# Geunwoo-Jeon/LarvaNet

Hardware: AMD Instinct MI355X
Metric: HR Mpixels/s (LarvaNet x4 multi-exit train step, 48x48 LR patches) (higher is better)
Workload: dtype f32; 1 GPU; LarvaNet x4 train_step_larva M4 B4,4,4,4 48ch, batch 16 of 3x48x48 -> 3x192x192 fp32 per GPU (BASELINE config 2); global_batch=16, parallelism=dp1, hip_graph=True

## Files before the change

### include/larva_hip.h

```cpp
#ifndef LARVA_HIP_H
#define LARVA_HIP_H

#include <stdint.h>

#ifdef __cplusplus
extern "C" {
#endif

int larva_abi_version(void);
const char* larva_error_string(int code);

long long larva_packed_weight_floats(int cout, int cin);
int larva_pack_weights(const float* w, float* wpk_fwd, float* wpk_bwd, int cout, int cin,
                       int w_cin_total, int w_cin_off, void* stream);

int larva_pack_weights_batch(const float* const* w, float* const* wpk_fwd, float* const* wpk_bwd,
                             const int* cout, const int* cin, const int* w_cin_total,
                             const int* w_cin_off, int njobs, void* stream);

int larva_step_prologue(const float* const* w, float* const* wpk_fwd, float* const* wpk_bwd, const int* cout,
                        const int* cin, const int* w_cin_total, const int* w_cin_off, int njobs, const float* x,
                        float* x16, float* base, int N, int C, int H, int W, void* stream);

int larva_conv3x3_fwd(const float* const* src, int n_src, int cin_per_src, const float* wpk,
                      const float* bias, const float* res0, const float* res1, const float* mask,
                      const float* base, float* out, int N, int cout, int H, int W, int relu,
                      int mode, void* stream);

int larva_conv3x3_fwd_pitched(const float* const* src, int n_src, int cin_per_src, const float* wpk,
                              const float* bias, const float* res0, const float* res1, const float* mask,
                              const float* base, float* out, int N, int cout, int H, int W, int pitch,
                              int relu, int mode, void* stream);

int larva_conv3x3_fwd_batch(int njobs, const float* const* src, int n_src, int cin_per_src,
                            const float* const* wpk, const float* const* bias, const float* const* res0,
                            const float* const* res1, const float* const* mask, const float* const* base,
                            float* const* out, int N, int cout, int H, int W, int pitch, int relu, int mode,
                            void* stream);

int larva_head_conv3_direct(const float* x, const float* w, const float* bias, float* out, int N, int cout,
                            int H, int W, int pitch, void* stream);

int larva_exit_l1_partials(int N, int H, int pitch);
int larva_conv3x3_exit_l1_batch(int njobs, const float* const* src, int n_src, int cin_per_src,
                                const float* const* wpk, const float* const* bias, const float* const* base,
                                const float* const* truth, float* const* out, float* const* grad,
                                float* const* partial, float gval, int N, int cout, int H, int W, int pitch,
                                void* stream);

int larva_strip_tile_table(int H, int W, int phase, unsigned* tab, int cap);
int larva_conv3x3_fwd_strips(const float* const* src, int n_src, int cin_per_src, const float* wpk,
                             const float* bias, const float* res0, const float* res1, const float* mask,
                             const float* base, float* out, int N, int cout, int H, int W, int pitch,
                             int relu, int mode, const unsigned* tile_tab, const unsigned* tile_tab_host,
                             int tiles_per_image, int plain_stores, void* stream);

int larva_conv3x3_fwd_tiled(const float* const* src, int n_src, int cin_per_src, const float* wpk,
                            const float* bias, const float* res0, const float* res1, const float* mask,
                            const float* base, float* out, int N, int cout, int H, int W, int pitch,
                            int relu, int mode, int tile_rows, void* stream);

long long larva_wgrad_partial_floats(int cout, int cin, int splits);
int larva_wgrad_cu_share(int cout, int cin);
int larva_conv3x3_wgrad(const float* const* dy, const float* const* x, float* const* partial,
                        float* const* dw, float* const* db, const int* cin_off,
                        const int* cin_valid, const int* w_cin_total, int njobs, int splits,
                        int N, int cout, int cin, int H, int W, void* stream);

int larva_wgrad_flat_max_splits(int njobs, int nwg, int tiles_per_layer);
int larva_conv3x3_wgrad_partial_flat(const float* const* dy, const float* const* x, float* const* partial,
                                     int njobs, int nwg, int N, int cout, int cin, int H, int W,
                                     int* splits_out, void* stream);
int larva_wgrad_flat_head_splits(int njobs, int nwg, int tiles_per_layer);
int larva_conv3x3_wgrad_partial_flat_head(const float* const* dy, const float* const* x, float* const* partial,
                                          int njobs, const float* head_dy, const float* head_x16, float* head_partial,
                                          int nwg, int N, int H, int W, int* splits_out, int* head_splits_out,
                                          void* stream);

int larva_conv3x3_wgrad_partial(const float* const* dy, const float* const* x, float* const* partial,
                                int njobs, int splits, int N, int cout, int cin, int H, int W,
                                int* splits_used, void* stream);
int larva_wgrad_reduce(const float* const* partial, float* const* dw, float* const* db,
                       const int* cin_off, const int* cin_valid, const int* w_cin_total,
                       const int* splits, const int* cout, const int* cin, int njobs, void* stream);

int larva_wgrad_reduce_with_loss(const float* const* partial, float* const* dw, float* const* db,
                                 const int* cin_off, const int* cin_valid, const int* w_cin_total,
                                 const int* splits, const int* cout, const int* cin, int njobs,
                                 const float* const* terms, const int* count, const float* scale, int nterms,
                                 float divisor, float* loss_out, void* stream);

int larva_bicubic4_fwd(const float* in, float* out, int N, int C, int H, int W, void* stream);
int larva_upsample4_fwd(const float* in, float* out, int N, int C, int H, int W, int mode, void* stream);

int larva_l1_workspace_floats(void);
int larva_l1_fwd(const float* a, const float* b, long long numel, float* partial, float* loss,
                 void* stream);
int larva_l1_bwd(const float* a, const float* b, const float* gout, long long numel, float* ga,
                 void* stream);
int larva_l1_bwd_unshuffle4(const float* a, const float* b, const float* gout, float gscale, float* ga, int N,
                            int C, int H, int W, void* stream);
int larva_sum_scalars(const float* const* terms, int n, float divisor, float* out, void* stream);
int larva_l1_partial(const float* a, const float* b, long long numel, float* partial, int* blocks_out,
                     void* stream);
int larva_loss_from_partials(const float* const* terms, const int* count, const float* scale, int n,
                             float divisor, float* out, void* stream);
int larva_loss_from_partials_to_host(const float* const* terms, const int* count, const float* scale, int n,
                                     float divisor, float* out, float* host_cell, void* stream);
int larva_loss_from_partials_to_host_seq(const float* const* terms, const int* count, const float* scale, int n,
                                         float divisor, float* out, float* host_cell, unsigned* dev_seq, void* stream);
int larva_host_cell_alloc(float** cell);
int larva_host_cell_free(float* cell);
int larva_l1_partial_grad(const float* a, const float* b, float gvalue, float gscale, float* partial,
                          int* blocks_out, float* grad, int N, int C, int H, int W, void* stream);
int larva_l1_partial_grad_batch(const float* const* a, const float* b, int n, float gvalue, float gscale,
                                float* const* partial, int* blocks_out, float* const* grad, int N, int C, int H,
                                int W, void* stream);

int larva_pixel_unshuffle4(const float* in, float* out, int N, int C, int H, int W, void* stream);

int larva_upsample_fwd(const float* in, float* out, int N, int C, int H, int W, int scale, int mode, void* stream);
int larva_pixel_shuffle_base(const float* y, const float* base, float* out, int N, int C, int cpad, int H, int W,
                             int pitch, int scale, void* stream);
int larva_pixel_unshuffle(const float* in, float* out, int N, int C, int cpad, int H, int W, int scale, void* stream);
int larva_l1_bwd_unshuffle(const float* a, const float* b, const float* gout, float gscale, float* ga, int N, int C,
                           int cpad, int H, int W, int scale, void* stream);
int larva_shuffle_l1_partial_grad(const float* y, const float* base, const float* truth, float gvalue, float gscale,
                                  float* partial, int* blocks_out, float* grad, float* out, int N, int C, int cpad, int H,
                                  int W, int scale, void* stream);

int larva_adamw_step(float* p, const float* g, float* m, float* v, const float* step_lr,
                     double beta1, double beta2, double eps, double weight_decay, float grad_scale,
                     long long n, void* stream);

int larva_adamw_step_host(float* p, const float* g, float* m, float* v, int step, double lr, double beta1,
                          double beta2, double eps, double weight_decay, float grad_scale, long long n,
                          void* stream);
int larva_adamw_step_host_copy(float* p, const float* g, float* m, float* v, int step, double lr, double beta1,
                               double beta2, double eps, double weight_decay, float grad_scale, long long n,
                               const float* copy_src, float* copy_dst, void* stream);

int larva_gather_patches(const unsigned char* data, const long long* offsets, const int* hw,
                         const int* draws, float* out, int B, int P, int mult, void* stream);

int larva_sqerr_u8(const float* out, const unsigned char* truth, int C, int H, int W, int TH, int TW,
                   unsigned long long* acc, void* stream);

int larva_u8_hwc_to_f32_chw(const unsigned char* in, float* out, int N, int H, int W, void* stream);
int larva_f32_chw_to_u8_hwc(const float* in, unsigned char* out, int N, int H, int W, void* stream);

long long larva_u8_metrics_workspace_bytes(int h, int w, int mode);
int larva_u8_metrics(const unsigned char* out, long long out_pitch, const unsigned char* truth, long long truth_pitch,
                     int y0, int x0, int h, int w, int mode, int want_ssim, void* workspace,
                     unsigned long long* result, void* stream);

long long larva_f16_packed_weight_halves(int cout, int cin);
int larva_f16_pack_weights(const float* w, uint16_t* wpk, int cout, int cin, void* stream);

int larva_f16_head(const float* x, const float* w, const float* bias, uint16_t* out, unsigned* flag, int N, int H,
                   int W, void* stream);

int larva_f16_conv3x3(const uint16_t* const* srcs, int nsrc, const uint16_t* wpk, const float* bias,
                      const uint16_t* res0, const uint16_t* res1, int relu, uint16_t* out, unsigned* flag, int N, int H,
                      int W, void* stream);

int larva_f16_conv3x3_shuffle_base(const uint16_t* src, const uint16_t* wpk, const float* bias, const float* base,
                                   float* out, int N, int H, int W, void* stream);

int larva_f16_conv3x3_shuffle_base_u8(const uint16_t* src, const uint16_t* wpk, const float* bias, const float* base,
                                      unsigned char* out, unsigned* flag, int N, int H, int W, void* stream);

int larva_f16_conv3x3_jobs(int njobs, const uint16_t* const* srcs, const uint16_t* const* wpks,
                           const float* const* biases, int relu, uint16_t* const* outs, unsigned* flag, int N, int H,
// ... 23 lines not shown
```

### larvanet_amd/autograd.py

```python
import contextlib
import os

import numpy as np
import torch

from . import kernels as K

_WGRAD_WORKGROUPS = 256


class PaddedWidth:

    current = None

    def __init__(self, w):
        self.w = int(w)

    def __enter__(self):
        self._prev = PaddedWidth.current
        PaddedWidth.current = self.w
        return self

    def __exit__(self, *exc):
        PaddedWidth.current = self._prev
# ... 10 lines not shown

class DualChain:

    enabled = False
    lazy_fwd = False
    lazy_bwd = False
    max_workgroups = 512
    _streams = {}
    _forked = False
    _keep = []

    @classmethod
    def wants(cls, n, h, p):
        if not cls.enabled or n < 2 or p % 4:
            return False
        if n * ((h + 2) // 3) * ((p + 47) // 48) > cls.max_workgroups:
            return False
        return K.strip_tile_table(h, p, torch.device("cuda", torch.cuda.current_device())) is not None

    _main = None

    @classmethod
    def _stream(cls, k):
        if k == 0 and cls._main is not None:
            return cls._main
        key = (torch.cuda.current_device(), k)
        if key not in cls._streams:
            cls._streams[key] = torch.cuda.Stream(device=key[0])
        return cls._streams[key]

    @classmethod
    def conv(cls, srcs, wpk, cout, forward=False, **kw):
        first = srcs if isinstance(srcs, torch.Tensor) else srcs[0]
        n, _, h, p = (int(v) for v in first.shape)
        if kw.get("logical_w") is not None or kw.get("shuffle") or not cls.wants(n, h, p):
            if cls._forked:
                cls.join()
            return K.conv3x3(srcs, wpk, cout, **kw)
        out = torch.empty((n, cout, h, p), device=first.device, dtype=torch.float32)
        cur = torch.cuda.current_stream()
        if not cls._forked:
            cls._main = cur
            for k in range(2):
                if cls._stream(k) != cur:
                    cls._stream(k).wait_stream(cur)
            cls._forked = True
        cls._keep.append(out)
        cls._keep.extend([srcs] if isinstance(srcs, torch.Tensor) else list(srcs))
        cls._keep.extend(t for t in (wpk, kw.get("bias"), kw.get("mask"), kw.get("res0"), kw.get("res1")) if t is not None)
        half = n // 2
        for k, rng in enumerate(((0, half), (half, n))):
            with torch.cuda.stream(cls._stream(k)):
                K.conv3x3(srcs, wpk, cout, out=out, images=rng, strips=2 if k else True, plain_stores=True, **kw)
        return out

    @classmethod
    def join(cls):
        try:
            if cls._forked:
                cur = torch.cuda.current_stream()
                for k in range(2):
                    if cls._stream(k) != cur:
                        cur.wait_stream(cls._stream(k))
        finally:
            cls._forked = False
            cls._main = None
            cls._keep.clear()

    @classmethod
    def reset(cls):
        cls._forked = False
        cls._main = None
        cls._keep.clear()

    @classmethod
    def end_of_node(cls, backward):
        if not (cls.lazy_bwd if backward else cls.lazy_fwd):
            cls.join()


class PackedConv:

    __slots__ = ("weight", "bias", "cin_pad", "slices", "_key", "_packs", "_bufs", "_prepacked", "grad_inplace",
                 "joint", "joint_slot", "cout_pad", "_pad")

    def __init__(self, weight, bias, cin_pad=None, slices=None, cout_pad=None):
        self.weight, self.bias, self.cin_pad = weight, bias, cin_pad
        self.cout_pad = cout_pad
        self._pad = None
        self.grad_inplace = False
        self.slices = slices
        self._key = None
        self._packs = None
        self._bufs = None
        self._prepacked = False
        self.joint = None
        self.joint_slot = 0

    def invalidate(self):
        self._key = None
        self._prepacked = False

    def _current_key(self):
        w = self.weight
        return (w.data_ptr(), w._version, str(w.device))

    def jobs(self):
        w = self.weight
        cout, cin_total = int(w.shape[0]), int(w.shape[1])
        dev = w.device
        if self.cout_pad is not None:
            w = self._padded(w)
            cout = self.cout_pad
        if self._bufs is None or self._bufs[0] != (w.data_ptr(), str(dev)):
            def buf(a, b):
                return torch.empty(K.packed_weight_floats(a, b), device=dev, dtype=torch.float32)
            if self.slices is None:
                cin_k = cin_total if self.cin_pad is None else self.cin_pad
                bwd = None if self.cin_pad is not None else \
                    (self.joint.view(self.joint_slot, dev) if self.joint is not None else buf(cin_k, cout))
                specs = [(buf(cout, cin_k), bwd, cin_k, 0)]
            else:
                specs = [(buf(cout, cin_total), None, cin_total, 0)]
                specs += [(buf(cout, c), buf(c, cout), c, o) for (o, c) in self.slices]
            self._bufs = ((w.data_ptr(), str(dev)), specs)
        wd = w.detach()
        return [(wd, f, b, cout, cin_k, off) for (f, b, cin_k, off) in self._bufs[1]]

    def _padded(self, w):
        rows = int(w.shape[0])
        if self._pad is None or self._pad[0].device != w.device or tuple(self._pad[0].shape[1:]) != tuple(w.shape[1:]):
            self._pad = (torch.zeros((self.cout_pad,) + tuple(w.shape[1:]), device=w.device, dtype=torch.float32),
                         torch.zeros(self.cout_pad, device=w.device, dtype=torch.float32))
        with torch.no_grad():
            self._pad[0][:rows].copy_(w.detach())
            self._pad[1][:rows].copy_(self.bias.detach())
        return self._pad[0]

    def padded_bias(self):
        return self._pad[1]

    def _mark_packed(self):
        self._packs = [(f, b) for (f, b, _, _) in self._bufs[1]]
        self._key = self._current_key()

    def refresh(self):
        if self._prepacked:
            self._prepacked = False
            return self
        if self._key != self._current_key() or (torch.is_grad_enabled() and self.weight.requires_grad):
            with torch.no_grad():
                K.pack_weights_batch(self.jobs())
            self._mark_packed()
        return self

    def get(self):
        if self._packs is None:
            self.refresh()
        return self._packs


class JointBwd:

    def __init__(self, first, second):
        cout, cin = int(first.weight.shape[0]), int(first.weight.shape[1])
        if tuple(second.weight.shape) != tuple(first.weight.shape) or first.slices or second.slices:
            raise RuntimeError("larvanet_amd: joint input gradients need two plain convs of one shape")
        self.floats = K.packed_weight_floats(cin, cout)
        self.cin = cin
        self._arena = None
        first.joint, first.joint_slot = self, 0
        second.joint, second.joint_slot = self, 1

    def arena(self, dev):
        if self._arena is None or self._arena.device != dev:
            self._arena = torch.empty(2 * self.floats, device=dev, dtype=torch.float32)
        return self._arena

    def view(self, slot, dev):
        return self.arena(dev)[slot * self.floats:(slot + 1) * self.floats]


class JointInputGrad:

    active = False
    _parked = {}

    @classmethod
    def reset(cls):
        cls._parked = {}

    @classmethod
    def can_park(cls, pc):
        return cls.active and pc.joint is not None and pc.joint_slot == 1

    @classmethod
    def park(cls, fea, dh, pc):
        cls._parked[fea.data_ptr()] = (dh, pc)

    @classmethod
    def take(cls, x, pc):
        if not cls._parked:
            return None
        hit = cls._parked.get(x.data_ptr())
        if hit is None or pc.joint is None or hit[1].joint is not pc.joint or pc.joint_slot != 0:
            return None
        del cls._parked[x.data_ptr()]
        return hit[0]


def step_prologue(pcs, x):
    jobs = []
    for pc in pcs:
        jobs += pc.jobs()
    N, C, H, W = (int(v) for v in x.shape)
    if len(jobs) > 64 or C > 16 or PaddedWidth.current is not None or not x.is_contiguous():
        return None
    x16 = StepScope.padded_input((N, 16, H, W), x.device)
    base = torch.empty((N, C, 4 * H, 4 * W), device=x.device, dtype=torch.float32)
    with torch.no_grad():
        K.step_prologue(jobs, x.detach(), x16, base)
    for pc in pcs:
        pc._mark_packed()
        pc._prepacked = True
    return x16, base


def pack_all(pcs):
    jobs = []
    for pc in pcs:
        jobs += pc.jobs()
    with torch.no_grad():
        K.pack_weights_batch(jobs)
    for pc in pcs:
        pc._mark_packed()
        pc._prepacked = True


class GradBucket:

    def __init__(self, module, pcs):
        params = [p for p in module.parameters() if p.requires_grad]
        total = sum(p.numel() for p in params)
        dev = params[0].device
        self.flat = torch.zeros(total, device=dev, dtype=torch.float32)
        off = 0
        self._pairs = []
        for p in params:
            view = self.flat[off:off + p.numel()].view_as(p)
            p.grad = view
            self._pairs.append((p, view))
            off += p.numel()
        owned = {id(p) for p in params}
        for pc in pcs:
            pc.grad_inplace = id(pc.weight) in owned and id(pc.bias) in owned

    def intact(self, module=None):
        return all(p.grad is view for p, view in self._pairs)

    def span(self, tensors):
        base = self.flat.data_ptr()
        lo, hi = self.flat.numel(), 0
        for t in tensors:
            off = (t.data_ptr() - base) // 4
            if off < 0 or off + t.numel() > self.flat.numel():
                return None
            lo, hi = min(lo, off), max(hi, off + t.numel())
        return (lo, hi) if hi > lo else None


def _targets(pc):
    if pc is not None and pc.grad_inplace and pc.weight.grad is not None and pc.bias.grad is not None:
        return pc.weight.grad, pc.bias.grad
    return None, None


def _splits(njobs, cout=48, cin=48):
    return max(1, _WGRAD_WORKGROUPS * K.wgrad_cu_share(cout, cin) // njobs)


class DeferredWgrad:

    active = False
    jobs_per_launch = 32
    _pending = {}

    @classmethod
    def push(cls, cout, cin, jobs):
        cls._pending.setdefault((cout, cin), []).extend(jobs)

    _late = []

    @classmethod
    def _launches(cls, split=False):
        pending, cls._pending = cls._pending, {}
        cap = max(1, min(cls.jobs_per_launch, K.max_wgrad_jobs())) if split else K.max_wgrad_jobs()
        out = []
        for (cout, cin), jobs in pending.items():
            jobs = sorted(jobs, key=lambda j: -j["dw"].data_ptr())
            out += [(cout, cin, jobs[i:i + cap]) for i in range(0, len(jobs), cap)]
        out.sort(key=lambda l: -max(j["dw"].data_ptr() for j in l[2]))
        return out

    pending_loss = None

    @classmethod
    def finish_loss(cls):
        job, cls.pending_loss = cls.pending_loss, None
        if job is not None:
            terms, scales, divisor, out = job
            out.copy_(K.loss_from_partials(terms, scales, divisor))

    @staticmethod
    def _issue(launches):
        reduce_jobs = []
        head = host = None
        heads = [l for l in launches if (l[0], l[1]) == (48, 16) and len(l[2]) == 1]
        hosts = [l for l in launches if (l[0], l[1]) == (48, 48)]
        if len(heads) == 1 and hosts and hosts[-1][2][0]["dy"].shape == heads[0][2][0]["dy"].shape:
            head, host = heads[0], hosts[-1]
        todo = [l for l in launches if l is not head]
        for launch in todo:
            cout, cin, chunk = launch
            extra = head[2][0] if launch is host else None
            res = K.conv3x3_wgrad_partial_flat(chunk, cout, cin, _WGRAD_WORKGROUPS, head=extra)
            if res is None and extra is not None:
                todo.append(head)
                extra = None
            if res is not None:
                reduce_jobs += [dict(j, partial=p, splits=s, cout=cout, cin=cin) for j, p, s in zip(chunk, *res)]
                if extra is not None:
                    reduce_jobs.append(dict(extra, partial=res[0][-1], splits=res[1][-1], cout=48, cin=16))
                continue
            parts, used = K.conv3x3_wgrad_partial(chunk, cout, cin, _splits(len(chunk), cout, cin))
            reduce_jobs += [dict(j, partial=p, splits=used, cout=cout, cin=cin) for j, p in zip(chunk, parts)]
        for i in range(0, len(reduce_jobs), 64):
            last = i + 64 >= len(reduce_jobs)
            loss, DeferredWgrad.pending_loss = (DeferredWgrad.pending_loss, None) if last else (None, DeferredWgrad.pending_loss)
            K.wgrad_reduce(reduce_jobs[i:i + 64], loss=loss)

    @classmethod
    def flush(cls, split=False):
        launches = cls._launches(split)
        n_early = max(1, len(launches) // 2) if split else len(launches)
        cls._issue(launches[:n_early])
        cls._late = launches[n_early:]
        if not split:
            return None
        return [t for _, _, chunk in launches[:n_early] for j in chunk for t in (j["dw"], j["db"]) if t is not None]

    @classmethod
    def has_late(cls):
        return bool(cls._late)

    @classmethod
    def late_targets(cls):
        return [t for _, _, chunk in cls._late for j in chunk for t in (j["dw"], j["db"]) if t is not None]

    @classmethod
    def flush_late(cls):
        late, cls._late = cls._late, []
        cls._issue(late)

    @classmethod
    def drop(cls):
        cls._pending = {}
        cls._late = []
        cls.pending_loss = None


class StepScope:

    depth = 0
    _padded = {}
    seed_grad = None
    early_loss = False

    @classmethod
    def padded_input(cls, shape, device):
        if cls.depth == 0:
            return torch.zeros(shape, device=device, dtype=torch.float32)
        key = (tuple(shape), str(device))
        buf = cls._padded.get(key)
        if buf is None:
            buf = cls._padded[key] = torch.zeros(shape, device=device, dtype=torch.float32)
        return buf

    def __init__(self, defer_wgrad=True, split_flush=False, joint_input_grads=True,
                 seed_grad=None, dual_chain=False, lazy_chain_joins=(False, False), early_loss=False):
        self.seed_grad_value = seed_grad
        self.early_loss_value = early_loss or False
        self.dual_chain = dual_chain
        self.lazy_chain_joins = lazy_chain_joins
        self.defer_wgrad = defer_wgrad
        self.split_flush = split_flush
        self.joint_input_grads = joint_input_grads
        self.early_targets = None

    def __enter__(self):
        gpu = torch.cuda.is_available()
        DeferredWgrad.active = bool(self.defer_wgrad) and gpu
        DeferredWgrad.drop()
        JointInputGrad.active = bool(self.joint_input_grads) and gpu
        JointInputGrad.reset()
        DualChain.enabled = bool(self.dual_chain) and gpu
        DualChain.lazy_fwd, DualChain.lazy_bwd = (bool(v) and DualChain.enabled for v in self.lazy_chain_joins)
        StepScope.depth += 1
        StepScope.seed_grad = self.seed_grad_value
        StepScope.early_loss = self.early_loss_value
        return self

    def __exit__(self, exc_type, *exc):
        try:
            DualChain.join()
            if exc_type is None:
                self.early_targets = DeferredWgrad.flush(split=self.split_flush)
                DeferredWgrad.finish_loss()
            else:
                DeferredWgrad.drop()
            if exc_type is None and JointInputGrad._parked:
                raise RuntimeError("larvanet_amd: an exit parked its input gradient but the next body never ran backward")
        finally:
            DualChain.reset()
            StepScope.depth -= 1
            StepScope.seed_grad = None
            StepScope.early_loss = False
            DeferredWgrad._pending = {}
            DualChain.enabled = DualChain.lazy_fwd = DualChain.lazy_bwd = False
            DeferredWgrad.active = False
            JointInputGrad.active = False
            JointInputGrad.reset()
        return False


def _wgrad(jobs, cout, cin, inplace=False):
    defer = inplace and DeferredWgrad.active
    out, batch = [], []
    for job in jobs:
        (dy, x, wshape, cin_off, cin_valid, dw_shared) = job[:6]
        db_shared = job[6] if len(job) > 6 else None
        dw = dw_shared if dw_shared is not None else torch.empty(wshape, device=dy.device, dtype=torch.float32)
        if db_shared is not None or not defer:
            db = db_shared if db_shared is not None else torch.empty((cout,), device=dy.device,
                                                                     dtype=torch.float32)
        else:
            db = None
        batch.append({"dy": dy, "x": x, "dw": dw, "db": db, "cin_off": cin_off, "cin_valid": cin_valid})
        out.append((dw, db))
    if defer:
        DeferredWgrad.push(cout, cin, batch)
        batch = []
    for i in range(0, len(batch), 16):
        chunk = batch[i:i + 16]
        K.conv3x3_wgrad(chunk, cout, cin, _splits(len(chunk), cout, cin))
    return out


LARGE_INFERENCE_PIXELS = 100000


def is_large_inference(n, h, w):
    return int(n) * int(h) * int(w) > LARGE_INFERENCE_PIXELS


def _head_direct_setting():
    v = os.environ.get("LARVA_HEAD_DIRECT", "auto")
    if v not in ("auto", "0", "1"):
        raise RuntimeError("larvanet_amd: LARVA_HEAD_DIRECT=%r (auto, 0 or 1)" % v)
    return {"0": False, "1": True}.get(v, "auto")


class HeadFn(torch.autograd.Function):

    direct = _head_direct_setting()
    rule_batch = None

    @staticmethod
    @contextlib.contextmanager
    def rule_batch_as(n):
        before, HeadFn.rule_batch = HeadFn.rule_batch, int(n)
        try:
            yield
        finally:
            HeadFn.rule_batch = before

    @staticmethod
    def forward(ctx, x, weight, bias, pc, x16=None, training=True):
        N, C, H, W = x.shape
        P = PaddedWidth.pitch_of(W) if _lw() is not None else W
        cout = int(weight.shape[0])
        training = bool(training) and bool(ctx.needs_input_grad[1] or ctx.needs_input_grad[2])
        want = HeadFn.direct if HeadFn.direct != "auto" else (not training and is_large_inference(HeadFn.rule_batch or N, H, W))
        use_direct = want and C == 3 and cout % 16 == 0
        if x16 is not None:
            pass
        elif training or not use_direct:
            x16 = StepScope.padded_input((N, 16, H, P), x.device)
            x16[:, :C, :, :W] = x
        if use_direct:
            out = K.head_conv3_direct(x, weight.detach(), bias.detach(), pitch=P)
        else:
            (fwd, _), = pc.get()
            out = DualChain.conv(x16, fwd, cout, forward=True, bias=bias.detach(), logical_w=_lw())
            DualChain.end_of_node(False)
        if x16 is not None:
            ctx.save_for_backward(x16)
        ctx.wshape = tuple(weight.shape)
        ctx.pc = pc
        return out

    @staticmethod
    def backward(ctx, dy):
# ... 374 lines not shown
```

### larvanet_amd/build.py

```python
import os
import shutil
import subprocess
import sys

CSRC = os.path.join(os.path.dirname(os.path.abspath(__file__)), "csrc")
LIB = os.path.join(CSRC, "liblarva_hip.so")
SOURCES = ["conv3x3_mfma.hip", "wgrad3x3_mfma.hip", "larva_pointwise.hip", "larva_scale.hip", "conv3x3_f16.hip",
           "larva_metrics.hip", "larva_ensemble.hip", "larva_downscale.hip"]
HEADERS = ["larva_common.h", "larva_bicubic.h", "larva_loss.h"]
FLAGS = ["--offload-arch=gfx950", "-O3", "-std=c++17", "-fPIC", "-Wall", "-Wno-unused-function"]


def _hipcc():
    exe = shutil.which("hipcc") or "/opt/rocm/bin/hipcc"
    if not os.path.exists(exe):
        raise RuntimeError("hipcc not found: the larvanet_amd HIP library cannot be built")
    return exe


def _check_ring_waits(temps, verbose):
    import glob
    asm = glob.glob(os.path.join(temps, "conv3x3_mfma-hip-amdgcn-*.s"))
    obj = os.path.join(temps, "conv3x3_mfma.o")
    if not asm or not os.path.exists(obj):
        raise RuntimeError("larvanet_amd.build: no device assembly from the conv kernel's compile (-save-temps)")
    checker = os.path.join(os.path.dirname(os.path.dirname(CSRC)), "tools", "check_aux_loads.py")
    r = subprocess.run([sys.executable, checker, asm[0]], stdout=subprocess.PIPE, stderr=subprocess.STDOUT)
    tail = r.stdout.decode(errors="replace").strip().splitlines()[-1:]
    if verbose:
        print("[larvanet_amd.build] ring waits vs emitted loads (tools/check_aux_loads.py):", " ".join(tail), flush=True)
    if r.returncode != 0:
        sys.stderr.write(r.stdout.decode(errors="replace"))
        raise RuntimeError("larvanet_amd.build: a counted vmcnt wait of conv3x3_mfma.hip does not match the loads hipcc emitted")
    os.replace(obj, os.path.join(CSRC, "conv3x3_mfma.o"))


def _stale(target, deps):
    if not os.path.exists(target):
        return True
    t = os.path.getmtime(target)
    return any(os.path.getmtime(d) > t for d in deps)


def build_extension(force=False, verbose=True):
    import tempfile
    hipcc = _hipcc()
    hdrs = [os.path.join(CSRC, h) for h in HEADERS]
    objs = []
    procs = []
    temps = None
    for src in SOURCES:
        s = os.path.join(CSRC, src)
        o = os.path.join(CSRC, src.replace(".hip", ".o"))
        objs.append(o)
        if force or _stale(o, [s] + hdrs):
            cmd = [hipcc] + FLAGS + ["-c", s, "-o", o]
            if src == "conv3x3_mfma.hip":
                temps = tempfile.mkdtemp(prefix="build_", dir=CSRC)
                cmd = [hipcc] + FLAGS + ["-save-temps=obj", "-c", s, "-o", os.path.join(temps, "conv3x3_mfma.o")]
            if verbose:
                print("[larvanet_amd.build]", " ".join(cmd), flush=True)
            procs.append((cmd, subprocess.Popen(cmd, stdout=subprocess.PIPE, stderr=subprocess.STDOUT)))
    try:
        for cmd, p in procs:
            out, _ = p.communicate()
            if p.returncode != 0:
                sys.stderr.write(out.decode(errors="replace"))
                raise RuntimeError("hipcc failed: " + " ".join(cmd))
        if temps is not None:
            _check_ring_waits(temps, verbose)
    finally:
        if temps is not None:
            shutil.rmtree(temps, ignore_errors=True)
    if force or procs or _stale(LIB, objs):
        cmd = [hipcc, "--offload-arch=gfx950", "-shared", "-fPIC", "-o", LIB] + objs
        if verbose:
            print("[larvanet_amd.build]", " ".join(cmd), flush=True)
        subprocess.run(cmd, check=True)
    return LIB


if __name__ == "__main__":
    build_extension(force="--force" in sys.argv)
    print(LIB)
```

### larvanet_amd/captured_step.py

```python
import contextlib

import torch

from .autograd import DeferredWgrad, DualChain


class LossCopy:

    def __init__(self):
        self.host = torch.empty((), dtype=torch.float32).pin_memory()
        self.stream = torch.cuda.Stream()
        self.done, self.fwd_done = torch.cuda.Event(), torch.cuda.Event()

    def start(self, loss):
        self.fwd_done.record()
        with torch.cuda.stream(self.stream):
            self.stream.wait_event(self.fwd_done)
            self.host.copy_(loss, non_blocking=True)
            self.done.record()

    def result(self):
        self.done.synchronize()
        return self.host.item()


class CapturedStep:

    def __init__(self, plugin, key, mode, handoff, input_tensor, truth_tensor):
        x, truth = input_tensor.clone(), truth_tensor.clone()
        side = torch.cuda.Stream()
        side.wait_stream(torch.cuda.current_stream())
        with torch.cuda.stream(side):
            for _ in range(2):
                plugin._zero_grad()
                plugin._step_body(x, truth)
                DeferredWgrad.flush_late()
        torch.cuda.current_stream().wait_stream(side)
        plugin._zero_grad()
        graph = torch.cuda.CUDAGraph()
        back = torch.cuda.CUDAGraph() if mode == "split" else None
        with contextlib.ExitStack() as capturing:
            capturing.enter_context(torch.cuda.graph(graph, capture_error_mode="thread_local"))

            def cut():
                DualChain.join()
                capturing.close()
                capturing.enter_context(torch.cuda.graph(back, pool=graph.pool(), capture_error_mode="thread_local"))
            loss, out, early_lo = plugin._step_body(x, truth, early_loss=handoff if mode == "poll" else bool(mode),
                                                    cut=cut if back is not None else None)
        late = None
        if DeferredWgrad.has_late():
            late = torch.cuda.CUDAGraph()
            with torch.cuda.graph(late, pool=graph.pool(), capture_error_mode="thread_local"):
                DeferredWgrad.flush_late()
        self.key, self.mode, self.handoff = key, mode, handoff
        self.static_in, self.static_truth = x, truth
        self.graph, self.back, self.late = graph, back, late
        self.loss, self.out, self.early_lo = loss, out, early_lo

    def stage(self, input_tensor, truth_tensor):
        for dst, src in ((self.static_in, input_tensor), (self.static_truth, truth_tensor)):
            if src.data_ptr() != dst.data_ptr():
                dst.copy_(src)

    def replay(self):
        if self.mode == "poll":
            self.handoff.expect()
        self.graph.replay()
        if self.back is not None:
            self.handoff.start(self.loss)
            self.back.replay()
        return self.loss, self.out, self.late.replay if self.late is not None else None

    def buffers(self, input_shape, truth_shape):
        fits = tuple(self.static_in.shape) == tuple(input_shape) and tuple(self.static_truth.shape) == tuple(truth_shape)
        return (self.static_in, self.static_truth) if fits else None
```

### larvanet_amd/csrc/conv3x3_mfma.hip

```cpp
#include "larva_common.h"
#include "larva_bicubic.h"
#include <hip/hip_ext.h>
#include <cstdlib>
#include <type_traits>

#ifndef LARVA_DIAG
#define LARVA_DIAG 0
#endif
constexpr int kWgPerCu = 2;
constexpr int kOperandDepth = 2;


#ifndef LARVA_DIAG_ONLY48
#define LARVA_DIAG_ONLY48 0
#endif

namespace larva {

#if defined(LARVA_DIAG) && (LARVA_DIAG & 32)
__device__ unsigned long long* g_stamps = nullptr;
#if LARVA_DIAG & 512
constexpr int kDiagWgPerSlot = 256;
__device__ int g_slot_of_launch = 0;
__device__ __forceinline__ void stamp_slot(unsigned long long* area, int k) {
// ... 847 lines not shown
    if (wave < 3) run_role<COUT, G, true, EPI, 1, 0, G::ROWS - 1>(a, smem, wave, wave, n, y0, x0, tid);
    else run_role<COUT, G, true, EPI, 3, G::ROWS - 1, 1>(a, smem, 0, wave, n, y0, x0, tid);
  } else if constexpr (G::ROWS == 5) {
    if (wave < 2) run_role<COUT, G, true, EPI, 1, 0, 3>(a, smem, wave, wave, n, y0, x0, tid);
    else if (wave == 2) run_role<COUT, G, true, EPI, 2, 3, 1>(a, smem, 0, wave, n, y0, x0, tid);
    else run_role<COUT, G, true, EPI, 2, 4, 1>(a, smem, 0, wave, n, y0, x0, tid);
  } else {
    if (wave < 2) run_role<COUT, G, true, EPI, 1, 0, 2>(a, smem, wave, wave, n, y0, x0, tid);
    else run_role<COUT, G, true, EPI, 1, 2, 2>(a, smem, wave - 2, wave, n, y0, x0, tid);
  }
}

template <int COUT, int EPI>
__global__ __launch_bounds__(320, kWgPerCu) void conv3x3_mfma_strip_kernel(ConvArgs a) {
  extern __shared__ __attribute__((aligned(16))) float smem[];
  stamp(0);
  fetch_args(a);
  const int tile = xcd_remap(blockIdx.x, a.nwg);
  const int n = div_by_magic(tile, a.magic_tx);
  const int slot = tile - n * a.tiles_x;
  unsigned e;
  if (a.tab_n) {
    const unsigned pair = (unsigned)a.tab16[slot >> 1];
    const unsigned h = (slot & 1) ? pair >> 16 : pair & 0xffffu;
    e = (h & 0xffu) | (((h >> 8) & 0x7fu) << 16) | ((h >> 15) << 31);
  } else {
    e = a.tile_tab[slot];
  }
  const int y0 = (int)(e & 0xfffu), x0 = (int)((e >> 12) & 0xfffu);
  const int tid = threadIdx.x;
  const int wave = __builtin_amdgcn_readfirstlane(tid >> 6);
  __builtin_amdgcn_s_setprio(1);
  if (e >> 31) strip_roles<COUT, EPI, GeoS5>(a, smem, wave, n, y0, x0, tid);
  else strip_roles<COUT, EPI, GeoS4>(a, smem, wave, n, y0, x0, tid);
}
template <int COUT>
constexpr size_t kStripLdsBytes = ConvCfg<COUT, GeoS5>::LDS_BYTES_DMA > ConvCfg<COUT, GeoS4>::LDS_BYTES_DMA ? ConvCfg<COUT, GeoS5>::LDS_BYTES_DMA
                                                                                                            : ConvCfg<COUT, GeoS4>::LDS_BYTES_DMA;
static_assert(kWgPerCu * kStripLdsBytes<48> <= 160 * 1024 && kWgPerCu * kStripLdsBytes<64> <= 160 * 1024, "strip workgroups per CU");

constexpr int kMaxConvJobs = 4;
struct ConvBatch {
  ConvArgs job[kMaxConvJobs];
};

template <int COUT, int EPI>
__global__ __launch_bounds__(ConvCfg<COUT>::THREADS_DMA, kWgPerCu) void conv3x3_mfma_batch_kernel(ConvBatch b) {
  extern __shared__ __attribute__((aligned(16))) float smem[];
  conv_tile<COUT, true, EPI>(b.job[blockIdx.y], smem);
}

constexpr int kMaxPackJobs = 64;

struct PackJob {
  const float* w;
  float* fwd;
  float* bwd;
  int cout, cin, w_cin_total, w_cin_off;
};

struct PackBatch {
  PackJob job[kMaxPackJobs];
};

__host__ __device__ constexpr int packed_floats(int cout, int cin) {
  return (cin / kCh) * 9 * kCh * cout_stride(cout);
}

constexpr int kPackTileCols = 64;
constexpr int kPackLd = kPackTileCols + 1;
constexpr int kPackTileFloats = 9 * kCh * kPackLd;

__host__ __device__ constexpr int pack_slots(int cout, int cin) { return cin / kCh + cout / kCh; }

__device__ __forceinline__ void pack_block(const PackJob& j, int slot, float* __restrict__ tile) {
  const int nfc = j.cin / kCh;
  const bool fwd = slot < nfc;
  const int chunk = fwd ? slot : slot - nfc;
  float* __restrict__ out = fwd ? j.fwd : j.bwd;
  if ((!fwd && chunk >= j.cout / kCh) || !out) return;
  const int cols = fwd ? j.cout : j.cin;
  const int cs = cout_stride(cols);
  const int tid = threadIdx.x;
  out += (size_t)chunk * 72 * cs;
  for (int c0 = 0; c0 < cs; c0 += kPackTileCols) {
    const int ncol = min(kPackTileCols, cols - c0);
    if (fwd) {
      for (int idx = tid; idx < ncol * 72; idx += 256) {
        const int c = idx / 72, r = idx - c * 72, k = r / 9, tap = r - k * 9;
        const int cin_abs = j.w_cin_off + chunk * kCh + k;
        tile[(tap * kCh + k) * kPackLd + c] =
            cin_abs < j.w_cin_total ? j.w[((size_t)(c0 + c) * j.w_cin_total + cin_abs) * 9 + tap] : 0.f;
      }
    } else {
      const int row = ncol * 9;
      for (int idx = tid; idx < kCh * row; idx += 256) {
        const int k = idx / row, rem = idx - k * row, c = rem / 9, tap = rem - c * 9;
        tile[((8 - tap) * kCh + k) * kPackLd + c] =
            j.w_cin_off + c0 + c < j.w_cin_total
                ? j.w[((size_t)(chunk * kCh + k) * j.w_cin_total + j.w_cin_off + c0) * 9 + rem] : 0.f;
      }
    }
    __syncthreads();
    const int wcols = min(kPackTileCols, cs - c0);
    const bool swz = cout_swizzled(cols);
    for (int idx = tid; idx < 72 * wcols; idx += 256) {
      const int r = idx / wcols, c = idx - r * wcols;
      const int col = swz ? ((c0 + c) ^ ((r & 1) << 4)) : c0 + c;
      out[r * cs + col] = c < ncol ? tile[r * kPackLd + c] : 0.f;
    }
    __syncthreads();
  }
}

__global__ __launch_bounds__(256) void pack_weights_batch_kernel(PackBatch b) {
  __shared__ float tile[kPackTileFloats];
  pack_block(b.job[blockIdx.y], blockIdx.x, tile);
}

constexpr int kPrologueBlocks = 192;
constexpr int kProloguePadSlices = 2, kPrologueBicSlices = 8;
struct PrologueArgs {
  PackBatch packs;
  int npack, slots;
  const float* x;
  float* x16;
  float* base;
  int N, C, H, W;
};

__global__ __launch_bounds__(256) void step_prologue_kernel(PrologueArgs a) {
  __shared__ float tile[kPackTileFloats];
  int blk = blockIdx.x;
  if (blk < a.npack * a.slots) {
    const int job = blk / a.slots;
    pack_block(a.packs.job[job], blk - job * a.slots, tile);
    return;
  }
  blk -= a.npack * a.slots;
  constexpr int nthr = kPrologueBlocks * 256;
  const int slice = blk / kPrologueBlocks, tid = (blk - slice * kPrologueBlocks) * 256 + threadIdx.x;
  const int nbic = a.base ? kPrologueBicSlices : 0;
  if (slice < nbic) {
    bicubic4_body(a.x, a.base, a.N * a.C, a.H, a.W, (long long)slice * nthr + tid, (long long)nthr * kPrologueBicSlices);
  } else {
    const int plane = a.H * a.W, per_img = a.C * plane, total = a.N * per_img;
    for (int i = (slice - nbic) * nthr + tid; i < total; i += nthr * kProloguePadSlices) {
      const int n = i / per_img, r = i - n * per_img;
      a.x16[(size_t)n * 16 * plane + r] = a.x[i];
    }
  }
}

struct LaunchTiming {
  hipEvent_t start, stop;
};

template <auto Kernel, typename Args>
static hipError_t launch(dim3 grid, dim3 block, size_t lds, hipStream_t stream, const LaunchTiming* tm, const Args& a) {
  static PerDeviceOnce lds_set;
  if (const hipError_t e = ensure_dynamic_lds(lds_set, reinterpret_cast<const void*>(Kernel), lds); e != hipSuccess) return e;
  if (tm)
    hipExtLaunchKernelGGL(Kernel, grid, block, lds, stream, tm->start, tm->stop, 0, a);
  else
    hipLaunchKernelGGL(Kernel, grid, block, lds, stream, a);
  return hipGetLastError();
}

template <int... E>
struct EpiSet {
  static constexpr bool has(int epi) { return ((epi == E) || ...); }
};
using EpiAll = EpiSet<kEpiPlain, kEpiRelu, kEpiMask, kEpiRes1, kEpiRes2, kEpiShuffle, kEpiShuffleBase>;
using EpiBatch48 = EpiSet<kEpiPlain, kEpiRelu, kEpiMask, kEpiRes1, kEpiRes2, kEpiShuffle, kEpiShuffleBase, kEpiShuffleL1>;
using EpiInference = EpiSet<kEpiPlain, kEpiRelu, kEpiRes1, kEpiRes2, kEpiShuffle, kEpiShuffleBase>;
using EpiRows4 = EpiInference;
using EpiPersist = EpiInference;

template <int... E, typename F>
static hipError_t with_epi(EpiSet<E...>, int epi, hipError_t absent, F&& f) {
  hipError_t r = absent;
  (void)((epi == E && (r = f(std::integral_constant<int, E>{}), true)) || ...);
  return r;
}

template <typename F>
static hipError_t with_cout(int cout, hipError_t absent, F&& f) {
  switch (cout) {
#if !LARVA_DIAG_ONLY48
    case 32: return f(std::integral_constant<int, 32>{});
    case 64: return f(std::integral_constant<int, 64>{});
#endif
// ... 404 lines not shown
```

### larvanet_amd/csrc/larva_common.h

```cpp
#pragma once
#include <hip/hip_runtime.h>
#include <stdint.h>

namespace larva {

typedef float f32x4 __attribute__((ext_vector_type(4)));

constexpr int kTileRows = 3;
constexpr int kTileCols = 48;
constexpr int kHaloRows = kTileRows + 2;
constexpr int kMaxSrc = 8;

constexpr int kRS = 56;

constexpr int kMaxDevices = 64;
inline int current_device_slot() {
  int d = 0;
  if (hipGetDevice(&d) != hipSuccess || d < 0) d = 0;
  return d < kMaxDevices ? d : kMaxDevices - 1;
}
struct PerDeviceOnce {
  bool done[kMaxDevices] = {};
};
inline hipError_t ensure_dynamic_lds(PerDeviceOnce& once, const void* kernel, size_t lds) {
  const int d = current_device_slot();
  if (once.done[d] && d != kMaxDevices - 1) return hipSuccess;
  const hipError_t e = hipFuncSetAttribute(kernel, hipFuncAttributeMaxDynamicSharedMemorySize, (int)lds);
  if (e == hipSuccess) once.done[d] = true;
  return e;
}
inline int device_cu_count() {
  static int cus[kMaxDevices] = {};
  const int d = current_device_slot();
  if (!cus[d] || d == kMaxDevices - 1) {
    int dev = 0, n = 0;
    if (hipGetDevice(&dev) != hipSuccess || hipDeviceGetAttribute(&n, hipDeviceAttributeMultiprocessorCount, dev) != hipSuccess || n <= 0)
      n = 256;
    cus[d] = n;
  }
  return cus[d];
}

__host__ __device__ constexpr int cout_stride(int cout) {
  return (cout % 32 == 16 || cout % 32 == 0) ? cout : cout + 16;
}
__host__ __device__ constexpr bool cout_swizzled(int cout) { return cout % 32 == 0; }

__device__ __forceinline__ int xcd_remap(int b, int nwg) {
  const int q = nwg >> 3, r = nwg & 7, xcd = b & 7;
  const int base = (xcd < r) ? xcd * (q + 1) : r * (q + 1) + (xcd - r) * q;
  return base + (b >> 3);
}

typedef int i32x4 __attribute__((ext_vector_type(4)));
typedef unsigned u32x4 __attribute__((ext_vector_type(4)));
constexpr unsigned kDmaZero = 0x80000000u;

__device__ __forceinline__ i32x4 dma_rsrc(const void* base) {
  const unsigned long long b = reinterpret_cast<unsigned long long>(base);
  i32x4 r;
  r[0] = __builtin_amdgcn_readfirstlane((int)(unsigned)b);
  r[1] = __builtin_amdgcn_readfirstlane((int)((unsigned)(b >> 32) & 0xffffu));
  r[2] = 0x7fffffff;
  r[3] = 0x00020000;
  return r;
}

template <bool SC1 = false>
__device__ __forceinline__ void lds_dma16_buf(i32x4 rsrc, unsigned voff, int soff_uniform, unsigned lds_addr_uniform) {
  unsigned keep;
  if constexpr (SC1) {
    asm volatile("s_mov_b32 %0, m0\n\ts_mov_b32 m0, %1\n\ts_nop 0\n\tbuffer_load_dwordx4 %2, %3, %4 offen sc1 lds\n\ts_mov_b32 m0, %0"
                 : "=&s"(keep)
                 : "s"(lds_addr_uniform), "v"(voff), "s"(rsrc), "s"(soff_uniform)
                 : "memory");
  } else {
    asm volatile("s_mov_b32 %0, m0\n\ts_mov_b32 m0, %1\n\ts_nop 0\n\tbuffer_load_dwordx4 %2, %3, %4 offen lds\n\ts_mov_b32 m0, %0"
                 : "=&s"(keep)
                 : "s"(lds_addr_uniform), "v"(voff), "s"(rsrc), "s"(soff_uniform)
                 : "memory");
  }
}

__device__ __forceinline__ unsigned lds_addr_of(const float* p) {
  return __builtin_amdgcn_readfirstlane((unsigned)(uintptr_t)((__attribute__((address_space(3))) const char*)p));
}

__device__ __forceinline__ unsigned quantize_u8(float v) { return (unsigned)fminf(fmaxf(rintf(v), 0.f), 255.f); }

struct rgb4_bytes {
  unsigned d[3];
};
__device__ __forceinline__ rgb4_bytes pack_rgb4(const f32x4 r, const f32x4 g, const f32x4 b) {
  unsigned q[12];
#pragma unroll
  for (int p = 0; p < 4; ++p) {
    q[3 * p + 0] = quantize_u8(r[p]);
    q[3 * p + 1] = quantize_u8(g[p]);
    q[3 * p + 2] = quantize_u8(b[p]);
  }
  rgb4_bytes o;
#pragma unroll
  for (int i = 0; i < 3; ++i) o.d[i] = q[4 * i] | (q[4 * i + 1] << 8) | (q[4 * i + 2] << 16) | (q[4 * i + 3] << 24);
  return o;
}

}
```

### larvanet_amd/csrc/larva_pointwise.hip

```cpp
#include "larva_common.h"
#include "larva_bicubic.h"
#include "larva_loss.h"

namespace larva {

__global__ void bicubic4_kernel(const float* __restrict__ in, float* __restrict__ out, int planes,
                                int H, int W) {
  bicubic4_body(in, out, planes, H, W, (long long)blockIdx.x * blockDim.x + threadIdx.x,
                (long long)gridDim.x * blockDim.x);
}

__global__ __launch_bounds__(256) void bicubic4_block_kernel(const float* __restrict__ in, float* __restrict__ out,
                                                              unsigned planes, unsigned H, unsigned W) {
  const unsigned total = planes * H * W;
  const unsigned i = blockIdx.x * 256u + threadIdx.x;
  if (i >= total) return;
  const unsigned x = i % W, t2 = i / W, y = t2 % H, p = t2 / H;
  const float* src = in + (size_t)p * H * W;
  int col[5];
#pragma unroll
  for (int c = 0; c < 5; ++c) col[c] = min(max((int)x - 2 + c, 0), (int)W - 1);
  float v[5][5];
#pragma unroll
  for (int r = 0; r < 5; ++r) {
    const float* row = src + (size_t)min(max((int)y - 2 + r, 0), (int)H - 1) * W;
#pragma unroll
    for (int c = 0; c < 5; ++c) v[r][c] = row[col[c]];
  }
  float wq[4][4];
  cubic_coeffs(0.625f, wq[0]);
  cubic_coeffs(0.875f, wq[1]);
  cubic_coeffs(0.125f, wq[2]);
  cubic_coeffs(0.375f, wq[3]);
  float h[5][4];
#pragma unroll
  for (int r = 0; r < 5; ++r)
#pragma unroll
    for (int jj = 0; jj < 4; ++jj) {
      float rowv = 0.f;
#pragma unroll
      for (int c = 0; c < 4; ++c) rowv += wq[jj][c] * v[r][(jj >> 1) + c];
      h[r][jj] = rowv;
    }
  float* o = out + ((size_t)p * (4 * H) + 4 * y) * (4 * W) + 4 * x;
#pragma unroll
  for (int ii = 0; ii < 4; ++ii) {
    f32x4 q;
#pragma unroll
    for (int jj = 0; jj < 4; ++jj) {
      float acc = 0.f;
#pragma unroll
      for (int r = 0; r < 4; ++r) acc += wq[ii][r] * h[(ii >> 1) + r][jj];
      q[jj] = acc;
    }
    *reinterpret_cast<f32x4*>(o + (size_t)ii * (4 * W)) = q;
  }
}

__global__ void bilinear4_kernel(const float* __restrict__ in, float* __restrict__ out, int planes, int H, int W) {
  const int HH = 4 * H;
  const long long total = (long long)planes * HH * W;
  for (long long i = (long long)blockIdx.x * blockDim.x + threadIdx.x; i < total; i += (long long)gridDim.x * blockDim.x) {
    const int x = (int)(i % W);
    const long long t2 = i / W;
    const int Y = (int)(t2 % HH);
    const int p = (int)(t2 / HH);
    const float* src = in + (size_t)p * H * W;
    const float sy = fmaxf(0.25f * ((float)Y + 0.5f) - 0.5f, 0.f);
    const int y0 = (int)sy, y1 = min(y0 + 1, H - 1);
    const float wy1 = sy - (float)y0, wy0 = 1.f - wy1;
    float v[2][3];
#pragma unroll
    for (int c = 0; c < 3; ++c) {
      const int xx = min(max(x - 1 + c, 0), W - 1);
      v[0][c] = src[(size_t)y0 * W + xx];
      v[1][c] = src[(size_t)y1 * W + xx];
    }
    f32x4 o;
#pragma unroll
    for (int jj = 0; jj < 4; ++jj) {
      const float sx = fmaxf(0.25f * ((float)(4 * x + jj) + 0.5f) - 0.5f, 0.f);
      const int x0 = (int)sx;
      const float wx1 = sx - (float)x0, wx0 = 1.f - wx1;
      const int c0 = x0 - (x - 1), c1 = min(x0 + 1, W - 1) - (x - 1);
      const float a0 = c0 == 0 ? v[0][0] : v[0][1], a1 = c1 == 0 ? v[0][0] : c1 == 1 ? v[0][1] : v[0][2];
// ... 245 lines not shown
#pragma unroll
  for (int o = 32; o > 0; o >>= 1) s += __shfl_xor(s, o);
  __shared__ float ws[4];
  if ((threadIdx.x & 63) == 0) ws[threadIdx.x >> 6] = s;
  __syncthreads();
  if (threadIdx.x == 0) partial[blockIdx.x] = (ws[0] + ws[1]) + (ws[2] + ws[3]);
}

struct L1Jobs {
  const float* a[8];
  float* partial[8];
  float* grad[8];
};
__global__ __launch_bounds__(256) void l1_partial_grad_batch_kernel(L1Jobs jobs, const float* __restrict__ b,
                                                                    long long numel, float g, int H, int W) {
  const float* __restrict__ a = jobs.a[blockIdx.y];
  float* __restrict__ partial = jobs.partial[blockIdx.y];
  float* __restrict__ grad = jobs.grad[blockIdx.y];
  float s = 0.f;
  const long long n4 = numel >> 2;
  const int HH = 4 * H;
  const size_t plane = (size_t)H * W;
  for (long long i = (long long)blockIdx.x * 256 + threadIdx.x; i < n4; i += (long long)gridDim.x * 256) {
    const f32x4 va = reinterpret_cast<const f32x4*>(a)[i];
    const f32x4 vb = reinterpret_cast<const f32x4*>(b)[i];
    s += fabsf(va[0] - vb[0]) + fabsf(va[1] - vb[1]) + fabsf(va[2] - vb[2]) + fabsf(va[3] - vb[3]);
    const int x = (int)(i % W);
    const long long t2 = i / W;
    const int Y = (int)(t2 % HH);
    const long long p = t2 / HH;
    float* o = grad + ((size_t)(p * 16 + 4 * (Y & 3)) * H + (Y >> 2)) * W + x;
#pragma unroll
    for (int e = 0; e < 4; ++e) {
      const float d = va[e] - vb[e];
      o[e * plane] = d > 0.f ? g : (d < 0.f ? -g : 0.f);
    }
  }
#pragma unroll
  for (int o = 32; o > 0; o >>= 1) s += __shfl_xor(s, o);
  __shared__ float ws[4];
  if ((threadIdx.x & 63) == 0) ws[threadIdx.x >> 6] = s;
  __syncthreads();
  if (threadIdx.x == 0) partial[blockIdx.x] = (ws[0] + ws[1]) + (ws[2] + ws[3]);
}

__global__ __launch_bounds__(256) void loss_from_partials_kernel(TermList l, float divisor, float* __restrict__ out,
                                                                 float* __restrict__ host_cell, unsigned* __restrict__ dev_seq) {
  loss_terms_block(l, divisor, out, host_cell, dev_seq);
}

struct ScalarList {
  const float* p[8];
  int n;
};
__global__ void sum_scalars_kernel(ScalarList l, float divisor, float* __restrict__ out) {
  if (threadIdx.x == 0 && blockIdx.x == 0) {
    float s = 0.f;
    for (int i = 0; i < l.n; ++i) s += l.p[i][0];
    out[0] = s / divisor;
  }
}

__global__ void pixel_unshuffle4_kernel(const float* __restrict__ in, float* __restrict__ out,
                                        int planes , int H, int W) {
  const int HH = 4 * H;
  const long long total = (long long)planes * HH * W;
  for (long long idx = (long long)blockIdx.x * blockDim.x + threadIdx.x; idx < total;
       idx += (long long)gridDim.x * blockDim.x) {
    const int x = (int)(idx % W);
    const long long t2 = idx / W;
    const int Y = (int)(t2 % HH);
    const int p = (int)(t2 / HH);
    const int y = Y >> 2, i = Y & 3;
    const f32x4 v = *reinterpret_cast<const f32x4*>(in + ((size_t)p * HH + Y) * (4 * W) + 4 * x);
    float* o = out + (((size_t)p * 16 + 4 * i) * H + y) * W + x;
    const size_t plane = (size_t)H * W;
    o[0] = v[0];
    o[plane] = v[1];
    o[2 * plane] = v[2];
    o[3 * plane] = v[3];
  }
}

struct AdamwCoef {
  float step_size, bc2_sqrt, decay;
};

__device__ __forceinline__ AdamwCoef adamw_coef_device(float step, float lr, double beta1, double beta2, float wd) {
  const double bc1 = 1.0 - pow(beta1, (double)step);
  const double bc2 = 1.0 - pow(beta2, (double)step);
  return AdamwCoef{(float)((double)lr / bc1), (float)sqrt(bc2), (float)(1.0 - (double)lr * (double)wd)};
}

__device__ __forceinline__ float rounded(float x) {
  asm volatile("" : "+v"(x));
  return x;
}

struct AdamwBetas {
  float beta2, omb1, omb2;
};

__device__ __forceinline__ void adamw_update(float& param, float& mi, float& vi, float grad, const AdamwCoef& c,
                                             const AdamwBetas& b, float eps) {
  mi = __fmaf_rn(b.omb1, rounded(grad - mi), mi);
  vi = __fmaf_rn(rounded(b.omb2 * grad), grad, rounded(vi * b.beta2));
  const float denom = rounded(__fdiv_rn(__fsqrt_rn(vi), c.bc2_sqrt)) + eps;
  param = rounded(param * c.decay) + rounded(__fdiv_rn(rounded(-c.step_size * mi), denom));
}

__global__ __launch_bounds__(256) void adamw_kernel(float* __restrict__ p, const float* __restrict__ g,
                                                    float* __restrict__ m, float* __restrict__ v,
                                                    const float* __restrict__ step_lr, AdamwCoef coef, double beta1,
                                                    double beta2, float eps, float wd, float gscale, long long n, int vec,
                                                    const float* __restrict__ copy_src, float* __restrict__ copy_dst) {
  if (copy_dst && blockIdx.x == 0 && threadIdx.x == 0) copy_dst[0] = copy_src[0];
  if (step_lr) coef = adamw_coef_device(step_lr[0], step_lr[1], beta1, beta2, wd);
  const AdamwBetas bt{(float)beta2, (float)(1.0 - beta1), (float)(1.0 - beta2)};
  const long long n4 = vec ? n >> 2 : 0;
  for (long long i = (long long)blockIdx.x * blockDim.x + threadIdx.x; i < n4; i += (long long)gridDim.x * blockDim.x) {
    f32x4 pp = reinterpret_cast<f32x4*>(p)[i], mm = reinterpret_cast<f32x4*>(m)[i], vv = reinterpret_cast<f32x4*>(v)[i];
    const f32x4 gg = reinterpret_cast<const f32x4*>(g)[i];
#pragma unroll
    for (int e = 0; e < 4; ++e) {
      float pe = pp[e], me = mm[e], ve = vv[e];
      adamw_update(pe, me, ve, __fmul_rn(gg[e], gscale), coef, bt, eps);
      pp[e] = pe; mm[e] = me; vv[e] = ve;
    }
    reinterpret_cast<f32x4*>(p)[i] = pp;
    reinterpret_cast<f32x4*>(m)[i] = mm;
    reinterpret_cast<f32x4*>(v)[i] = vv;
  }
  for (long long i = (n4 << 2) + (long long)blockIdx.x * blockDim.x + threadIdx.x; i < n;
       i += (long long)gridDim.x * blockDim.x) {
    float pp = p[i], mm = m[i], vv = v[i];
    adamw_update(pp, mm, vv, __fmul_rn(g[i], gscale), coef, bt, eps);
    p[i] = pp; m[i] = mm; v[i] = vv;
  }
}

static int adamw_vec_ok(const void* p, const void* g, const void* m, const void* v) {
  return ((reinterpret_cast<uintptr_t>(p) | reinterpret_cast<uintptr_t>(g) | reinterpret_cast<uintptr_t>(m) |
           reinterpret_cast<uintptr_t>(v)) & 15) == 0;
}

__global__ void gather_patches_kernel(const unsigned char* __restrict__ data,
                                      const long long* __restrict__ offsets, const int* __restrict__ hw,
                                      const int* __restrict__ draws, float* __restrict__ out, int B, int P,
                                      int mult) {
  const long long total = (long long)B * 3 * P * P;
  for (long long idx = (long long)blockIdx.x * blockDim.x + threadIdx.x; idx < total;
       idx += (long long)gridDim.x * blockDim.x) {
    const int j = (int)(idx % P);
    long long t = idx / P;
    const int i = (int)(t % P); t /= P;
    const int c = (int)(t % 3);
    const int b = (int)(t / 3);
    const int* d = draws + 5 * b;
    const int img = d[0], x0 = d[1] * mult, y0 = d[2] * mult, k = d[3] & 3, flip = d[4];
    const int H = hw[2 * img], W = hw[2 * img + 1];
    const int jj = flip ? P - 1 - j : j;
    int si, sj;
    if (k == 0) { si = i; sj = jj; }
    else if (k == 1) { si = jj; sj = P - 1 - i; }
    else if (k == 2) { si = P - 1 - i; sj = P - 1 - jj; }
    else { si = P - 1 - jj; sj = i; }
    out[idx] = (float)data[offsets[img] + ((long long)c * H + (y0 + si)) * W + (x0 + sj)];
  }
}

__global__ __launch_bounds__(256) void sqerr_u8_kernel(const float* __restrict__ out,
                                                       const unsigned char* __restrict__ truth, int C, int H,
                                                       int W, int TH, int TW,
                                                       unsigned long long* __restrict__ acc) {
  const long long total = (long long)C * H * W;
  unsigned long long s = 0;
  for (long long i = (long long)blockIdx.x * blockDim.x + threadIdx.x; i < total;
       i += (long long)gridDim.x * blockDim.x) {
    const int x = (int)(i % W);
    const long long t = i / W;
    const int y = (int)(t % H);
    const int c = (int)(t / H);
    const float q = fminf(fmaxf(rintf(out[i]), 0.f), 255.f);
    const int d = (int)truth[((size_t)c * TH + y) * TW + x] - (int)q;
    s += (unsigned long long)(d * d);
  }
#pragma unroll
  for (int o = 32; o > 0; o >>= 1) s += __shfl_xor(s, o);
  if ((threadIdx.x & 63) == 0) atomicAdd(acc, s);
}

static inline int grid_for(long long work, int block) {
// ... 196 lines not shown
  void* p = nullptr;
  hipError_t e = hipHostMalloc(&p, 64, hipHostMallocCoherent | hipHostMallocMapped);
  if (e != hipSuccess) return (int)e;
  *cell = static_cast<float*>(p);
  (*cell)[0] = __builtin_nanf("");
  reinterpret_cast<unsigned*>(p)[1] = 0u;
  return 0;
}

int larva_host_cell_free(float* cell) {
  if (!cell) return 0;
  (void)hipDeviceSynchronize();
  return (int)hipHostFree(cell);
}

int larva_l1_bwd_unshuffle4(const float* a, const float* b, const float* gout, float gscale, float* ga, int N,
                            int C, int H, int W, void* stream) {
  if (!a || !b || !gout || !ga || N <= 0 || C <= 0 || H <= 0 || W <= 0) return (int)hipErrorInvalidValue;
  if ((reinterpret_cast<uintptr_t>(a) | reinterpret_cast<uintptr_t>(b)) & 15) return (int)hipErrorInvalidValue;
  const long long work = (long long)N * C * 4 * H * W;
  const float inv = 1.0f / (float)(work * 4);
  hipLaunchKernelGGL(l1_bwd_unshuffle4_kernel, dim3(grid_for(work, 256)), dim3(256), 0, (hipStream_t)stream, a, b,
                     gout, gscale, inv, ga, N * C, H, W);
  return (int)hipGetLastError();
}


int larva_sum_scalars(const float* const* terms, int n, float divisor, float* out, void* stream) {
  if (!terms || n < 1 || n > 8 || !out) return (int)hipErrorInvalidValue;
  ScalarList l{};
  for (int i = 0; i < n; ++i) {
    if (!terms[i]) return (int)hipErrorInvalidValue;
    l.p[i] = terms[i];
  }
  l.n = n;
  hipLaunchKernelGGL(sum_scalars_kernel, dim3(1), dim3(64), 0, (hipStream_t)stream, l, divisor, out);
  return (int)hipGetLastError();
}

int larva_l1_bwd(const float* a, const float* b, const float* gout, long long numel, float* ga,
                 void* stream) {
  if (!a || !b || !gout || !ga || numel <= 0) return (int)hipErrorInvalidValue;
  if ((reinterpret_cast<uintptr_t>(a) | reinterpret_cast<uintptr_t>(b) | reinterpret_cast<uintptr_t>(ga)) & 15)
    return (int)hipErrorInvalidValue;
  hipLaunchKernelGGL(l1_bwd_kernel, dim3(grid_for(numel / 4, 256)), dim3(256), 0, (hipStream_t)stream, a, b,
                     gout, 1.0f / (float)numel, numel, ga);
  return (int)hipGetLastError();
}

int larva_pixel_unshuffle4(const float* in, float* out, int N, int C, int H, int W, void* stream) {
  if (!in || !out || N <= 0 || C <= 0 || H <= 0 || W <= 0) return (int)hipErrorInvalidValue;
  const long long work = (long long)N * C * 4 * H * W;
  hipLaunchKernelGGL(pixel_unshuffle4_kernel, dim3(grid_for(work, 256)), dim3(256), 0, (hipStream_t)stream, in,
                     out, N * C, H, W);
  return (int)hipGetLastError();
}

int larva_adamw_step(float* p, const float* g, float* m, float* v, const float* step_lr, double beta1,
                     double beta2, double eps, double weight_decay, float grad_scale, long long n,
                     void* stream) {
  if (!p || !g || !m || !v || !step_lr || n <= 0) return (int)hipErrorInvalidValue;
  hipLaunchKernelGGL(adamw_kernel, dim3(grid_for((n + 3) / 4, 256)), dim3(256), 0, (hipStream_t)stream, p, g, m, v,
                     step_lr, AdamwCoef{}, beta1, beta2, (float)eps, (float)weight_decay, grad_scale, n, adamw_vec_ok(p, g, m, v),
                     (const float*)nullptr,
                     (float*)nullptr);
  return (int)hipGetLastError();
}

int larva_adamw_step_host_copy(float* p, const float* g, float* m, float* v, int step, double lr, double beta1,
                               double beta2, double eps, double weight_decay, float grad_scale, long long n,
                               const float* copy_src, float* copy_dst, void* stream);

int larva_adamw_step_host(float* p, const float* g, float* m, float* v, int step, double lr, double beta1,
                          double beta2, double eps, double weight_decay, float grad_scale, long long n,
                          void* stream) {
  return larva_adamw_step_host_copy(p, g, m, v, step, lr, beta1, beta2, eps, weight_decay, grad_scale, n, nullptr, nullptr,
                                    stream);
}

int larva_adamw_step_host_copy(float* p, const float* g, float* m, float* v, int step, double lr, double beta1,
                               double beta2, double eps, double weight_decay, float grad_scale, long long n,
                               const float* copy_src, float* copy_dst, void* stream) {
  if (!p || !g || !m || !v || n <= 0 || step < 1 || (copy_dst && !copy_src)) return (int)hipErrorInvalidValue;
  const double bc1 = 1.0 - pow(beta1, (double)step), bc2 = 1.0 - pow(beta2, (double)step);
  const AdamwCoef coef{(float)(lr / bc1), (float)sqrt(bc2), (float)(1.0 - lr * weight_decay)};
  hipLaunchKernelGGL(adamw_kernel, dim3(grid_for((n + 3) / 4, 256)), dim3(256), 0, (hipStream_t)stream, p, g, m, v,
                     (const float*)nullptr, coef, beta1, beta2, (float)eps, (float)weight_decay, grad_scale, n, adamw_vec_ok(p, g, m, v),
                     copy_src, copy_dst);
  return (int)hipGetLastError();
}

int larva_gather_patches(const unsigned char* data, const long long* offsets, const int* hw,
                         const int* draws, float* out, int B, int P, int mult, void* stream) {
  if (!data || !offsets || !hw || !draws || !out || B <= 0 || P <= 0 || mult <= 0) return (int)hipErrorInvalidValue;
  hipLaunchKernelGGL(gather_patches_kernel, dim3(grid_for((long long)B * 3 * P * P, 256)), dim3(256), 0,
                     (hipStream_t)stream, data, offsets, hw, draws, out, B, P, mult);
  return (int)hipGetLastError();
}

int larva_sqerr_u8(const float* out, const unsigned char* truth, int C, int H, int W, int TH, int TW,
                   unsigned long long* acc, void* stream) {
  if (!out || !truth || !acc || C <= 0 || H <= 0 || W <= 0 || TH < H || TW < W) return (int)hipErrorInvalidValue;
  hipLaunchKernelGGL(sqerr_u8_kernel, dim3(grid_for((long long)C * H * W, 256)), dim3(256), 0, (hipStream_t)stream,
                     out, truth, C, H, W, TH, TW, acc);
  return (int)hipGetLastError();
}

static bool image_shape_ok(int N, int H, int W) {
  return N > 0 && H > 0 && W > 0 && (long long)N * H * W * 3 < (1ll << 40);
}

int larva_u8_hwc_to_f32_chw(const unsigned char* in, float* out, int N, int H, int W, void* stream) {
  if (!in || !out || !image_shape_ok(N, H, W)) return (int)hipErrorInvalidValue;
  const long long HW = (long long)H * W;
  if (u8_vec_ok(in, out, HW)) {
    const long long total = N * (HW / 4);
    hipLaunchKernelGGL(u8_hwc_to_f32_chw_kernel<true>, dim3(grid_for(total, 256)), dim3(256), 0, (hipStream_t)stream, in,
                       out, HW, total);
  } else {
    const long long total = N * HW;
    hipLaunchKernelGGL(u8_hwc_to_f32_chw_kernel<false>, dim3(grid_for(total, 256)), dim3(256), 0, (hipStream_t)stream, in,
                       out, HW, total);
  }
  return (int)hipGetLastError();
}

int larva_f32_chw_to_u8_hwc(const float* in, unsigned char* out, int N, int H, int W, void* stream) {
  if (!in || !out || !image_shape_ok(N, H, W)) return (int)hipErrorInvalidValue;
  const long long HW = (long long)H * W;
  if (u8_vec_ok(in, out, HW)) {
    const long long total = N * (HW / 4);
    hipLaunchKernelGGL(f32_chw_to_u8_hwc_kernel<true>, dim3(grid_for(total, 256)), dim3(256), 0, (hipStream_t)stream, in,
                       out, HW, total);
  } else {
    const long long total = N * HW;
    hipLaunchKernelGGL(f32_chw_to_u8_hwc_kernel<false>, dim3(grid_for(total, 256)), dim3(256), 0, (hipStream_t)stream, in,
                       out, HW, total);
  }
  return (int)hipGetLastError();
}

const char* larva_error_string(int code) { return hipGetErrorString((hipError_t)code); }

int larva_abi_version(void) { return 5; }

}
```

### larvanet_amd/csrc/wgrad3x3_mfma.hip

```cpp
#include "larva_common.h"
#include "larva_loss.h"

#include <type_traits>

#ifndef WG_DIAG
#define WG_DIAG 0
#endif
constexpr int kWgMinGaps = 6;


namespace larva {

constexpr int kMaxJobs = 64;

struct WgradJob {
  const float* dy;
  const float* x;
  float* partial;
};

struct WgradBatch {
  WgradJob job[kMaxJobs];
  int N, H, W;
  int tiles_x, tiles_y;
  int vec_ok;
  int njobs;
  short first_wg[kMaxJobs];
  WgradJob head;
  int head_units;
  int head_first_wg;
  int halves;
#if defined(LARVA_DIAG) && (LARVA_DIAG & 512)
  unsigned long long* diag_area;
#endif
};

#if defined(LARVA_DIAG) && (LARVA_DIAG & 512)
__device__ __forceinline__ void wstamp(unsigned long long* area, int k) {
  if (!area || threadIdx.x != 0 || blockIdx.x >= 256) return;
  unsigned long long* p = area + (size_t)blockIdx.x * 4;
  p[k] = __builtin_amdgcn_s_memrealtime();
  if (k == 0) {
    const unsigned hw = __builtin_amdgcn_s_getreg((31 << 11) | 4);
    const unsigned xcc = __builtin_amdgcn_s_getreg((31 << 11) | 20);
    p[2] = (unsigned long long)hw | ((unsigned long long)xcc << 32);
  }
}
#define WSTAMP(b, k) wstamp((b).diag_area, (k))
#else
#define WSTAMP(b, k) ((void)0)
#endif

constexpr int kHeadCost10 = 6;
__host__ __device__ constexpr int flat_head_units(int tiles) { return (tiles * kHeadCost10 + 9) / 10; }

template <int COUT, int CIN>
struct WgCfg {
  static constexpr int CT = COUT / 16;
  static constexpr int NB = (CIN / 16) * 9;
  static constexpr int NBW = (NB + 3) / 4;
  static constexpr int PSD = 146;
  static constexpr int PSX = 278;
  static constexpr int DY_FLOATS = COUT * PSD;
  static constexpr int X_FLOATS = CIN * PSX + 8;
  static constexpr size_t LDS_BYTES = (DY_FLOATS + X_FLOATS) * sizeof(float);
  static constexpr int DY_SLOTS = COUT * kTileRows * (kTileCols / 4);
  static constexpr int X_SLOTS = CIN * kHaloRows * (kRS / 4);
  static constexpr int DY_ITERS = (DY_SLOTS + 255) / 256;
  static constexpr int X_ITERS = (X_SLOTS + 255) / 256;
  static constexpr int PARTIAL_FLOATS = NB * CT * 256 + COUT;
};

template <int COUT, int CIN>
struct WgStaging {
  f32x4 dy[WgCfg<COUT, CIN>::DY_ITERS];
  f32x4 x[WgCfg<COUT, CIN>::X_ITERS];
  uint32_t ok_dy, ok_x;
};

template <int COUT, int CIN, bool VEC>
__device__ __forceinline__ void wg_load(const WgradBatch& b, const WgradJob& j, int tile, int tid,
                                        WgStaging<COUT, CIN>& st) {
  using C = WgCfg<COUT, CIN>;
  const int tx = tile % b.tiles_x;
// ... 734 lines not shown
template <int COUT, int CIN>
__global__ __launch_bounds__(256, 1) void wgrad3x3_pipe_flat_kernel(WgradBatch b) {
  extern __shared__ __attribute__((aligned(16))) float smem[];
  WSTAMP(b, 0);
  const int tid = threadIdx.x;
  const int wave = __builtin_amdgcn_readfirstlane(tid >> 6);
  const int w = blockIdx.x, nwg = gridDim.x;
  const int total = b.N * b.tiles_x * b.tiles_y;
  const long long T = (long long)total * b.njobs;
  const long long G = T + b.head_units;
  const int g0 = __builtin_amdgcn_readfirstlane((int)((G * w) / nwg));
  const int g1 = __builtin_amdgcn_readfirstlane((int)((G * (w + 1)) / nwg));
  int g = g0;
  const int g_end = min(g1, (int)T);
  int jb = __builtin_amdgcn_readfirstlane(g / total);
  while (g < g_end) {
    const int base = jb * total;
    const int seg_end = min(g_end, base + total);
    const WgradJob& j = b.job[jb];
    float* part = j.partial + (size_t)(w - b.first_wg[jb]) * pipe_image_floats<COUT, CIN>(b);
    wg_pipe_waves<COUT, CIN>(b, j, smem, g - base, seg_end - base, part, tid, wave);
    __syncthreads();
    g = seg_end;
    ++jb;
  }
  if (b.head_units > 0 && g1 > (int)T) {
    using H = WgCfg<COUT, 16>;
    const long long p0 = max(g0, (int)T) - T, p1 = g1 - T;
    const int h_begin = __builtin_amdgcn_readfirstlane((int)(p0 * total / b.head_units));
    const int h_end = __builtin_amdgcn_readfirstlane((int)(p1 * total / b.head_units));
    float* part = b.head.partial + (size_t)(w - b.head_first_wg) * H::PARTIAL_FLOATS;
    if constexpr (WgPipe<COUT, 16>::FITS) {
      static_assert(WgPipe<COUT, 16>::LDS_BYTES <= WgPipe<COUT, CIN>::LDS_BYTES, "the head's tile buffers fit the launch's LDS");
      const size_t plane = (size_t)b.H * b.W;
      const PipeSeg seg{b.head.dy, b.head.x, 16 * plane, part, part + H::NB * H::CT * 256};
      wg_pipe_pass<COUT, 16>(b, seg, smem, h_begin, h_end, tid, wave);
    } else {
      constexpr int NB = H::NB;
      constexpr int W0 = (NB + 3) / 4, W1 = (NB + 2) / 4, W2 = (NB + 1) / 4, W3 = NB / 4;
      if (wave == 0) wg_role_range<COUT, 16, true, 0, W0>(b, b.head, smem, h_begin, h_end, part, tid, true);
      else if (wave == 1) wg_role_range<COUT, 16, true, W0, W1>(b, b.head, smem, h_begin, h_end, part, tid, false);
      else if (wave == 2) wg_role_range<COUT, 16, true, W0 + W1, W2>(b, b.head, smem, h_begin, h_end, part, tid, false);
      else wg_role_range<COUT, 16, true, W0 + W1 + W2, W3>(b, b.head, smem, h_begin, h_end, part, tid, false);
    }
  }
#if defined(LARVA_DIAG) && (LARVA_DIAG & 512)
  __syncthreads();
  asm volatile("s_waitcnt vmcnt(0)" ::: "memory");
  WSTAMP(b, 1);
#endif
}

template <int COUT, int CIN>
constexpr int kWgradPerCu = (COUT * CIN <= 32 * 32 && 2 * WgCfg<COUT, CIN>::LDS_BYTES <= 160 * 1024) ? 2 : 1;

template <int COUT, int CIN, bool VEC>
__global__ __launch_bounds__(256, (kWgradPerCu<COUT, CIN>)) void wgrad3x3_kernel(WgradBatch b) {
  using C = WgCfg<COUT, CIN>;
  extern __shared__ __attribute__((aligned(16))) float smem[];
  const WgradJob& j = b.job[blockIdx.y];
  const int tid = threadIdx.x;
  const int wave = __builtin_amdgcn_readfirstlane(tid >> 6);
  const int split = blockIdx.x, splits = gridDim.x;
  constexpr int NB = C::NB;
  constexpr int W0 = (NB + 3) / 4, W1 = (NB + 2) / 4, W2 = (NB + 1) / 4, W3 = NB / 4;
  if (wave == 0) wg_role<COUT, CIN, VEC, 0, W0>(b, j, smem, split, splits, tid, true);
  else if (wave == 1) wg_role<COUT, CIN, VEC, W0, W1>(b, j, smem, split, splits, tid, false);
  else if (wave == 2) wg_role<COUT, CIN, VEC, W0 + W1, W2>(b, j, smem, split, splits, tid, false);
  else wg_role<COUT, CIN, VEC, W0 + W1 + W2, W3>(b, j, smem, split, splits, tid, false);
}

struct ReduceJob {
  const float* partial;
  float* dw;
  float* db;
  int cin_off;
  int cin_valid;
  int w_cin_total;
  int splits;
  int cout, cin;
};

constexpr int kMaxReduceJobs = 64;

struct ReduceBatch {
  ReduceJob job[kMaxReduceJobs];
  int njobs;
  TermList loss_terms;
  float loss_divisor;
  float* loss_out;
};

constexpr int kReduceRow = 16 * 9 + 1;
constexpr int kReduceColumnwiseAbove = 16;

__device__ __forceinline__ void reduce_columnwise(const ReduceJob& j) {
  __shared__ f32x4 meet[3][64];
  const int ct_n = j.cout / 16, nb = (j.cin / 16) * 9;
  const int n_w = nb * ct_n * 256;
  const int pf = n_w + j.cout;
  const int col = threadIdx.x & 63, wave = threadIdx.x >> 6;
  const int i = (blockIdx.x * 64 + col) * 4;
  if (blockIdx.x * 256 >= pf) return;
  f32x4 s = {0.f, 0.f, 0.f, 0.f};
  if (i < pf) {
    const float* p = j.partial + i;
    int k = wave;
    for (; k + 28 < j.splits; k += 32) {
      f32x4 v[8];
#pragma unroll
      for (int u = 0; u < 8; ++u) v[u] = *reinterpret_cast<const f32x4*>(p + (size_t)(k + 4 * u) * pf);
#pragma unroll
      for (int u = 0; u < 8; ++u) s += v[u];
    }
    for (; k < j.splits; k += 4) s += *reinterpret_cast<const f32x4*>(p + (size_t)k * pf);
  }
  if (wave) meet[wave - 1][col] = s;
  __syncthreads();
  if (wave || i >= pf) return;
  s = (s + meet[0][col]) + (meet[1][col] + meet[2][col]);
  if (i < n_w) {
    const int lane = (i >> 2) & 63;
    const int t = i >> 8;
    const int c = t % ct_n, bi = t / ct_n;
    const int cit = bi / 9, tap = bi % 9;
    const int co0 = c * 16 + (lane >> 4) * 4;
    const int ci = cit * 16 + (lane & 15);
    if (ci < j.cin_valid) {
#pragma unroll
      for (int r = 0; r < 4; ++r) j.dw[((size_t)(co0 + r) * j.w_cin_total + j.cin_off + ci) * 9 + tap] = s[r];
    }
  } else if (j.db) {
#pragma unroll
    for (int r = 0; r < 4; ++r) j.db[i - n_w + r] = s[r];
  }
}

__global__ __launch_bounds__(256) void wgrad_reduce_kernel(ReduceBatch rb) {
  if ((int)blockIdx.y == rb.njobs) {
    if (blockIdx.x == 0) loss_terms_block(rb.loss_terms, rb.loss_divisor, rb.loss_out);
    return;
  }
  __shared__ float tile[16 * kReduceRow];
  const ReduceJob& j = rb.job[blockIdx.y];
  if (j.splits > kReduceColumnwiseAbove) return reduce_columnwise(j);
  const int ct_n = j.cout / 16;
  const int c = blockIdx.x % ct_n, cit = blockIdx.x / ct_n;
  if (cit >= j.cin / 16) return;
  const int n_w = (j.cin / 16) * 9 * ct_n * 256;
  const int pf = n_w + j.cout;
  const int tid = threadIdx.x;
  if (tid < 192) {
    const int lane = tid & 63, tap0 = tid >> 6;
    f32x4 s[3];
    const float* p[3];
#pragma unroll
    for (int u = 0; u < 3; ++u) {
      s[u] = f32x4{0.f, 0.f, 0.f, 0.f};
      p[u] = j.partial + ((size_t)((cit * 9 + tap0 + 3 * u) * ct_n + c) * 256 + lane * 4);
    }
    int k = 0;
    for (; k + 8 <= j.splits; k += 8) {
      f32x4 v[3][8];
#pragma unroll
      for (int u = 0; u < 3; ++u)
#pragma unroll
        for (int q = 0; q < 8; ++q) v[u][q] = *reinterpret_cast<const f32x4*>(p[u] + (size_t)(k + q) * pf);
#pragma unroll
      for (int u = 0; u < 3; ++u)
#pragma unroll
        for (int q = 0; q < 8; ++q) s[u] += v[u][q];
    }
    for (; k < j.splits; ++k)
#pragma unroll
      for (int u = 0; u < 3; ++u) s[u] += *reinterpret_cast<const f32x4*>(p[u] + (size_t)k * pf);
    const int co = (lane >> 4) * 4, ci = lane & 15;
#pragma unroll
    for (int u = 0; u < 3; ++u)
#pragma unroll
      for (int r = 0; r < 4; ++r) tile[(co + r) * kReduceRow + ci * 9 + tap0 + 3 * u] = s[u][r];
  } else if (cit == 0 && j.db && tid < 192 + 16) {
    const float* p = j.partial + n_w + c * 16 + (tid - 192);
    float sb = 0.f;
    for (int k = 0; k < j.splits; ++k) sb += p[(size_t)k * pf];
    j.db[c * 16 + (tid - 192)] = sb;
  }
  __syncthreads();
  const int ci_n = min(16, j.cin_valid - cit * 16);
#pragma unroll
  for (int e = 0; e < 9; ++e) {
    const int idx = e * 256 + tid, co = idx / 144, rem = idx - co * 144;
    if (rem < ci_n * 9)
      j.dw[((size_t)(c * 16 + co) * j.w_cin_total + j.cin_off + cit * 16) * 9 + rem] = tile[co * kReduceRow + rem];
  }
}

template <int COUT, int CIN>
constexpr int kPipeHalves = WgPipe<COUT, CIN>::FITS ? 1 : ((CIN == 64 && WgPipe<COUT, 32>::FITS) ? 2 : 0);

template <int COUT, int CIN>
static hipError_t launch_wgrad(const WgradBatch& b, int njobs, int splits, hipStream_t stream) {
  using C = WgCfg<COUT, CIN>;
  using P = WgPipe<COUT, CIN>;
  if constexpr (kPipeHalves<COUT, CIN> == 2) {
    if (b.vec_ok) {
      using P2 = WgPipe<COUT, CIN / 2>;
      static PerDeviceOnce lds_half;
      if (const hipError_t e = ensure_dynamic_lds(lds_half, reinterpret_cast<const void*>(wgrad3x3_pipe_kernel<COUT, CIN / 2>), P2::LDS_BYTES);
          e != hipSuccess)
        return e;
      WgradBatch b2 = b;
      b2.halves = 2;
      hipLaunchKernelGGL((wgrad3x3_pipe_kernel<COUT, CIN / 2>), dim3(splits, njobs), dim3(256), P2::LDS_BYTES, stream, b2);
      return hipGetLastError();
    }
  }
  static PerDeviceOnce lds_a, lds_b, lds_c;
  if (const hipError_t e = ensure_dynamic_lds(lds_a, reinterpret_cast<const void*>(wgrad3x3_kernel<COUT, CIN, true>), C::LDS_BYTES); e != hipSuccess)
    return e;
  if (const hipError_t e = ensure_dynamic_lds(lds_b, reinterpret_cast<const void*>(wgrad3x3_kernel<COUT, CIN, false>), C::LDS_BYTES); e != hipSuccess)
    return e;
  if constexpr (P::FITS) {
    if (const hipError_t e = ensure_dynamic_lds(lds_c, reinterpret_cast<const void*>(wgrad3x3_pipe_kernel<COUT, CIN>), P::LDS_BYTES); e != hipSuccess)
      return e;
  }
  if constexpr (P::FITS) {
    if (b.vec_ok) {
      hipLaunchKernelGGL((wgrad3x3_pipe_kernel<COUT, CIN>), dim3(splits, njobs), dim3(256), P::LDS_BYTES, stream, b);
      return hipGetLastError();
    }
  }
  if (b.vec_ok)
    hipLaunchKernelGGL((wgrad3x3_kernel<COUT, CIN, true>), dim3(splits, njobs), dim3(256), C::LDS_BYTES, stream, b);
  else
    hipLaunchKernelGGL((wgrad3x3_kernel<COUT, CIN, false>), dim3(splits, njobs), dim3(256), C::LDS_BYTES, stream, b);
  return hipGetLastError();
}

template <int COUT, int CIN>
static hipError_t launch_wgrad_flat(const WgradBatch& b, int nwg, hipStream_t stream) {
  using P = WgPipe<COUT, CIN>;
  static_assert(P::FITS, "the flat launch exists for the pipelined kernel only");
  static PerDeviceOnce lds_set;
  if (const hipError_t e = ensure_dynamic_lds(lds_set, reinterpret_cast<const void*>(wgrad3x3_pipe_flat_kernel<COUT, CIN>), P::LDS_BYTES);
      e != hipSuccess)
    return e;
  hipLaunchKernelGGL((wgrad3x3_pipe_flat_kernel<COUT, CIN>), dim3(nwg), dim3(256), P::LDS_BYTES, stream, b);
  return hipGetLastError();
}

}

using namespace larva;

extern "C" {

int larva_wgrad_flat_max_splits(int njobs, int nwg, int tiles_per_layer) {
  if (njobs < 1 || nwg < 1 || tiles_per_layer < 1) return 0;
  const long long G = (long long)njobs * tiles_per_layer;
  if (nwg > G) nwg = (int)G;
  const long long smallest = G / nwg;
  return (int)((tiles_per_layer + smallest - 1) / smallest + 1);
}

int larva_wgrad_flat_head_splits(int njobs, int nwg, int tiles_per_layer);

#if defined(LARVA_DIAG) && (LARVA_DIAG & 512)
static int g_wdiag_next = -1, g_wdiag_cap = 0;
static unsigned long long* g_wdiag_base = nullptr;
#endif
static int wgrad_flat_impl(const float* const* dy, const float* const* x, float* const* partial, int njobs,
                           const float* head_dy, const float* head_x16, float* head_partial, int nwg, int N, int cout,
                           int cin, int H, int W, int* splits_out, int* head_splits_out, void* stream) {
  if (njobs < 1 || njobs > kMaxJobs || nwg < 1 || nwg > 32767 || N <= 0 || H <= 0 || W <= 0 || !splits_out)
    return (int)hipErrorInvalidValue;
  if (!((cout == 48 && cin == 48) || (cout == 32 && cin == 32) || (cout == 64 && cin == 64)) || W % 4)
    return (int)hipErrorNotSupported;
// ... 107 lines not shown
    return (int)hipErrorInvalidValue;
  WgradBatch b{};
  bool aligned = (W % 4 == 0);
  for (int i = 0; i < njobs; ++i) {
    if (!dy[i] || !x[i] || !partial[i]) return (int)hipErrorInvalidValue;
    b.job[i] = WgradJob{dy[i], x[i], partial[i]};
    aligned = aligned && ((reinterpret_cast<uintptr_t>(dy[i]) & 15) == 0) &&
              ((reinterpret_cast<uintptr_t>(x[i]) & 15) == 0);
  }
  b.N = N; b.H = H; b.W = W;
  b.tiles_x = (W + kTileCols - 1) / kTileCols;
  b.tiles_y = (H + kTileRows - 1) / kTileRows;
  b.vec_ok = aligned ? 1 : 0;
  const int total = N * b.tiles_x * b.tiles_y;
  if (splits > total) splits = total;
  if (splits_used) *splits_used = splits;
  hipStream_t s = (hipStream_t)stream;
  hipError_t e;
  if (cout == 48 && cin == 48) e = launch_wgrad<48, 48>(b, njobs, splits, s);
  else if (cout == 48 && cin == 16) e = launch_wgrad<48, 16>(b, njobs, splits, s);
  else if (cout == 32 && cin == 32) e = launch_wgrad<32, 32>(b, njobs, splits, s);
  else if (cout == 64 && cin == 64) e = launch_wgrad<64, 64>(b, njobs, splits, s);
  else if (cout == 32 && cin == 16) e = launch_wgrad<32, 16>(b, njobs, splits, s);
  else if (cout == 64 && cin == 16) e = launch_wgrad<64, 16>(b, njobs, splits, s);
  else if (cout == 48 && cin == 32) e = launch_wgrad<48, 32>(b, njobs, splits, s);
  else if (cout == 48 && cin == 64) e = launch_wgrad<48, 64>(b, njobs, splits, s);
  else if (cout == 32 && cin == 48) e = launch_wgrad<32, 48>(b, njobs, splits, s);
  else return (int)hipErrorInvalidValue;
  return (int)e;
}

static int reduce_launch(const float* const* partial, float* const* dw, float* const* db, const int* cin_off,
                         const int* cin_valid, const int* w_cin_total, const int* splits, const int* cout, const int* cin,
                         int njobs, const TermList* loss, float divisor, float* loss_out, void* stream) {
  if (njobs < 1 || njobs > kMaxReduceJobs) return (int)hipErrorInvalidValue;
  ReduceBatch rb{};
  int pf_max = 0;
  for (int i = 0; i < njobs; ++i) {
    if (!partial[i] || !dw[i] || splits[i] < 1 || cout[i] <= 0 || cin[i] <= 0 || cout[i] % 16 || cin[i] % 16)
      return (int)hipErrorInvalidValue;
    rb.job[i] = ReduceJob{partial[i], dw[i], db ? db[i] : nullptr, cin_off[i], cin_valid[i], w_cin_total[i],
                          splits[i], cout[i], cin[i]};
    const int pf = splits[i] > kReduceColumnwiseAbove
                       ? (((cin[i] / 16) * 9 * (cout[i] / 16) * 256 + cout[i]) / 4 + 63) / 64
                       : (cout[i] / 16) * (cin[i] / 16);
    pf_max = pf > pf_max ? pf : pf_max;
  }
  rb.njobs = njobs;
  if (loss) {
    rb.loss_terms = *loss;
    rb.loss_divisor = divisor;
    rb.loss_out = loss_out;
  }
  hipLaunchKernelGGL(wgrad_reduce_kernel, dim3(pf_max, njobs + (loss ? 1 : 0)), dim3(256), 0,
                     (hipStream_t)stream, rb);
  return (int)hipGetLastError();
}

int larva_wgrad_reduce(const float* const* partial, float* const* dw, float* const* db,
                       const int* cin_off, const int* cin_valid, const int* w_cin_total,
                       const int* splits, const int* cout, const int* cin, int njobs, void* stream) {
  return reduce_launch(partial, dw, db, cin_off, cin_valid, w_cin_total, splits, cout, cin, njobs, nullptr, 1.f, nullptr,
                       stream);
}

int larva_wgrad_reduce_with_loss(const float* const* partial, float* const* dw, float* const* db,
                                 const int* cin_off, const int* cin_valid, const int* w_cin_total,
                                 const int* splits, const int* cout, const int* cin, int njobs,
                                 const float* const* terms, const int* count, const float* scale, int nterms,
                                 float divisor, float* loss_out, void* stream) {
  if (!terms || !count || !scale || nterms < 1 || nterms > 8 || !loss_out) return (int)hipErrorInvalidValue;
  TermList l{};
  for (int i = 0; i < nterms; ++i) {
    if (!terms[i] || count[i] < 1) return (int)hipErrorInvalidValue;
    l.p[i] = terms[i];
    l.count[i] = count[i];
    l.scale[i] = scale[i];
  }
  l.n = nterms;
  return reduce_launch(partial, dw, db, cin_off, cin_valid, w_cin_total, splits, cout, cin, njobs, &l, divisor, loss_out,
                       stream);
}

int larva_conv3x3_wgrad(const float* const* dy, const float* const* x, float* const* partial,
                        float* const* dw, float* const* db, const int* cin_off,
                        const int* cin_valid, const int* w_cin_total, int njobs, int splits,
                        int N, int cout, int cin, int H, int W, void* stream) {
  int used = 0;
  int rc = larva_conv3x3_wgrad_partial(dy, x, partial, njobs, splits, N, cout, cin, H, W, &used, stream);
  if (rc) return rc;
  int sp[kMaxJobs], co[kMaxJobs], ci[kMaxJobs];
  for (int i = 0; i < njobs; ++i) { sp[i] = used; co[i] = cout; ci[i] = cin; }
  return larva_wgrad_reduce(partial, dw, db, cin_off, cin_valid, w_cin_total, sp, co, ci, njobs, stream);
}

}
```

### larvanet_amd/hip_lib.py

```python
import ctypes
import os

_HERE = os.path.dirname(os.path.abspath(__file__))
LIB_PATH = os.path.join(_HERE, "csrc", "liblarva_hip.so")

_c_float_p = ctypes.c_void_p
_c_pp = ctypes.POINTER(ctypes.c_void_p)
_c_int_p = ctypes.POINTER(ctypes.c_int)

SIGNATURES = {
    "larva_abi_version": (ctypes.c_int, []),
    "larva_error_string": (ctypes.c_char_p, [ctypes.c_int]),
    "larva_packed_weight_floats": (ctypes.c_longlong, [ctypes.c_int, ctypes.c_int]),
    "larva_pack_weights": (ctypes.c_int, [_c_float_p, _c_float_p, _c_float_p, ctypes.c_int, ctypes.c_int,
                                          ctypes.c_int, ctypes.c_int, ctypes.c_void_p]),
    "larva_pack_weights_batch": (ctypes.c_int, [_c_pp, _c_pp, _c_pp, _c_int_p, _c_int_p, _c_int_p, _c_int_p,
                                                ctypes.c_int, ctypes.c_void_p]),
    "larva_step_prologue": (ctypes.c_int, [_c_pp, _c_pp, _c_pp, _c_int_p, _c_int_p, _c_int_p, _c_int_p, ctypes.c_int,
                                           _c_float_p, _c_float_p, _c_float_p, ctypes.c_int, ctypes.c_int, ctypes.c_int,
                                           ctypes.c_int, ctypes.c_void_p]),
    "larva_conv3x3_fwd": (ctypes.c_int, [_c_pp, ctypes.c_int, ctypes.c_int, _c_float_p, _c_float_p,
                                         _c_float_p, _c_float_p, _c_float_p, _c_float_p, _c_float_p,
                                         ctypes.c_int, ctypes.c_int, ctypes.c_int, ctypes.c_int,
                                         ctypes.c_int, ctypes.c_int, ctypes.c_void_p]),
    "larva_conv3x3_fwd_pitched": (ctypes.c_int, [_c_pp, ctypes.c_int, ctypes.c_int, _c_float_p, _c_float_p,
                                                 _c_float_p, _c_float_p, _c_float_p, _c_float_p, _c_float_p,
                                                 ctypes.c_int, ctypes.c_int, ctypes.c_int, ctypes.c_int,
                                                 ctypes.c_int, ctypes.c_int, ctypes.c_int, ctypes.c_void_p]),
    "larva_conv3x3_fwd_batch": (ctypes.c_int, [ctypes.c_int, _c_pp, ctypes.c_int, ctypes.c_int, _c_pp, _c_pp, _c_pp, _c_pp,
                                               _c_pp, _c_pp, _c_pp, ctypes.c_int, ctypes.c_int, ctypes.c_int,
                                               ctypes.c_int, ctypes.c_int, ctypes.c_int, ctypes.c_int, ctypes.c_void_p]),
    "larva_conv3x3_fwd_tiled": (ctypes.c_int, [_c_pp, ctypes.c_int, ctypes.c_int, _c_float_p, _c_float_p,
                                               _c_float_p, _c_float_p, _c_float_p, _c_float_p, _c_float_p,
                                               ctypes.c_int, ctypes.c_int, ctypes.c_int, ctypes.c_int,
                                               ctypes.c_int, ctypes.c_int, ctypes.c_int, ctypes.c_int, ctypes.c_void_p]),
    "larva_conv3x3_fwd_strips": (ctypes.c_int, [_c_pp, ctypes.c_int, ctypes.c_int, _c_float_p, _c_float_p,
                                                _c_float_p, _c_float_p, _c_float_p, _c_float_p, _c_float_p,
                                                ctypes.c_int, ctypes.c_int, ctypes.c_int, ctypes.c_int,
                                                ctypes.c_int, ctypes.c_int, ctypes.c_int, ctypes.c_void_p,
                                                ctypes.POINTER(ctypes.c_uint), ctypes.c_int, ctypes.c_int, ctypes.c_void_p]),
    "larva_head_conv3_direct": (ctypes.c_int, [_c_float_p, _c_float_p, _c_float_p, _c_float_p, ctypes.c_int, ctypes.c_int,
                                               ctypes.c_int, ctypes.c_int, ctypes.c_int, ctypes.c_void_p]),
    "larva_exit_l1_partials": (ctypes.c_int, [ctypes.c_int, ctypes.c_int, ctypes.c_int]),
    "larva_conv3x3_exit_l1_batch": (ctypes.c_int, [ctypes.c_int, _c_pp, ctypes.c_int, ctypes.c_int, _c_pp, _c_pp, _c_pp, _c_pp,
                                                   _c_pp, _c_pp, _c_pp, ctypes.c_float, ctypes.c_int, ctypes.c_int,
                                                   ctypes.c_int, ctypes.c_int, ctypes.c_int, ctypes.c_void_p]),
    "larva_strip_tile_table": (ctypes.c_int, [ctypes.c_int, ctypes.c_int, ctypes.c_int, ctypes.POINTER(ctypes.c_uint),
                                              ctypes.c_int]),
    "larva_wgrad_partial_floats": (ctypes.c_longlong, [ctypes.c_int, ctypes.c_int, ctypes.c_int]),
    "larva_conv3x3_wgrad": (ctypes.c_int, [_c_pp, _c_pp, _c_pp, _c_pp, _c_pp, _c_int_p, _c_int_p, _c_int_p,
                                           ctypes.c_int, ctypes.c_int, ctypes.c_int, ctypes.c_int,
                                           ctypes.c_int, ctypes.c_int, ctypes.c_int, ctypes.c_void_p]),
    "larva_conv3x3_wgrad_partial": (ctypes.c_int, [_c_pp, _c_pp, _c_pp, ctypes.c_int, ctypes.c_int, ctypes.c_int,
                                                   ctypes.c_int, ctypes.c_int, ctypes.c_int, ctypes.c_int,
                                                   _c_int_p, ctypes.c_void_p]),
    "larva_wgrad_flat_head_splits": (ctypes.c_int, [ctypes.c_int, ctypes.c_int, ctypes.c_int]),
    "larva_conv3x3_wgrad_partial_flat_head": (ctypes.c_int, [_c_pp, _c_pp, _c_pp, ctypes.c_int, _c_float_p, _c_float_p,
                                                             _c_float_p, ctypes.c_int, ctypes.c_int, ctypes.c_int,
                                                             ctypes.c_int, _c_int_p, _c_int_p, ctypes.c_void_p]),
    "larva_wgrad_flat_max_splits": (ctypes.c_int, [ctypes.c_int, ctypes.c_int, ctypes.c_int]),
    "larva_conv3x3_wgrad_partial_flat": (ctypes.c_int, [_c_pp, _c_pp, _c_pp, ctypes.c_int, ctypes.c_int, ctypes.c_int,
                                                        ctypes.c_int, ctypes.c_int, ctypes.c_int, ctypes.c_int,
                                                        _c_int_p, ctypes.c_void_p]),
    "larva_wgrad_reduce": (ctypes.c_int, [_c_pp, _c_pp, _c_pp, _c_int_p, _c_int_p, _c_int_p, _c_int_p, _c_int_p,
                                          _c_int_p, ctypes.c_int, ctypes.c_void_p]),
    "larva_wgrad_reduce_with_loss": (ctypes.c_int, [_c_pp, _c_pp, _c_pp, _c_int_p, _c_int_p, _c_int_p, _c_int_p, _c_int_p,
                                                    _c_int_p, ctypes.c_int, _c_pp, _c_int_p, _c_float_p, ctypes.c_int,
                                                    ctypes.c_float, _c_float_p, ctypes.c_void_p]),
    "larva_adamw_step_host_copy": (ctypes.c_int, [_c_float_p, _c_float_p, _c_float_p, _c_float_p, ctypes.c_int,
                                                  ctypes.c_double, ctypes.c_double, ctypes.c_double, ctypes.c_double,
                                                  ctypes.c_double, ctypes.c_float, ctypes.c_longlong, _c_float_p, _c_float_p,
                                                  ctypes.c_void_p]),
    "larva_upsample4_fwd": (ctypes.c_int, [_c_float_p, _c_float_p, ctypes.c_int, ctypes.c_int, ctypes.c_int,
                                           ctypes.c_int, ctypes.c_int, ctypes.c_void_p]),
    "larva_bicubic4_fwd": (ctypes.c_int, [_c_float_p, _c_float_p, ctypes.c_int, ctypes.c_int, ctypes.c_int,
                                          ctypes.c_int, ctypes.c_void_p]),
    "larva_l1_workspace_floats": (ctypes.c_int, []),
    "larva_l1_fwd": (ctypes.c_int, [_c_float_p, _c_float_p, ctypes.c_longlong, _c_float_p, _c_float_p,
                                    ctypes.c_void_p]),
    "larva_l1_bwd": (ctypes.c_int, [_c_float_p, _c_float_p, _c_float_p, ctypes.c_longlong, _c_float_p,
                                    ctypes.c_void_p]),
    "larva_l1_bwd_unshuffle4": (ctypes.c_int, [_c_float_p, _c_float_p, _c_float_p, ctypes.c_float, _c_float_p,
                                               ctypes.c_int, ctypes.c_int, ctypes.c_int, ctypes.c_int, ctypes.c_void_p]),
    "larva_l1_partial": (ctypes.c_int, [_c_float_p, _c_float_p, ctypes.c_longlong, _c_float_p, _c_int_p,
                                        ctypes.c_void_p]),
    "larva_l1_partial_grad": (ctypes.c_int, [_c_float_p, _c_float_p, ctypes.c_float, ctypes.c_float, _c_float_p,
                                             _c_int_p, _c_float_p, ctypes.c_int, ctypes.c_int, ctypes.c_int,
                                             ctypes.c_int, ctypes.c_void_p]),
    "larva_l1_partial_grad_batch": (ctypes.c_int, [_c_pp, _c_float_p, ctypes.c_int, ctypes.c_float, ctypes.c_float, _c_pp,
                                                   _c_int_p, _c_pp, ctypes.c_int, ctypes.c_int, ctypes.c_int,
                                                   ctypes.c_int, ctypes.c_void_p]),
    "larva_loss_from_partials_to_host": (ctypes.c_int, [_c_pp, _c_int_p, _c_float_p, ctypes.c_int, ctypes.c_float,
                                                        _c_float_p, _c_float_p, ctypes.c_void_p]),
    "larva_loss_from_partials_to_host_seq": (ctypes.c_int, [_c_pp, _c_int_p, _c_float_p, ctypes.c_int, ctypes.c_float,
                                                            _c_float_p, _c_float_p, ctypes.c_void_p, ctypes.c_void_p]),
    "larva_host_cell_alloc": (ctypes.c_int, [ctypes.POINTER(ctypes.c_void_p)]),
    "larva_host_cell_free": (ctypes.c_int, [_c_float_p]),
    "larva_loss_from_partials": (ctypes.c_int, [_c_pp, _c_int_p, _c_float_p, ctypes.c_int, ctypes.c_float,
                                                _c_float_p, ctypes.c_void_p]),
    "larva_sum_scalars": (ctypes.c_int, [_c_pp, ctypes.c_int, ctypes.c_float, _c_float_p, ctypes.c_void_p]),
    "larva_upsample_fwd": (ctypes.c_int, [_c_float_p, _c_float_p, ctypes.c_int, ctypes.c_int, ctypes.c_int, ctypes.c_int,
                                          ctypes.c_int, ctypes.c_int, ctypes.c_void_p]),
    "larva_pixel_shuffle_base": (ctypes.c_int, [_c_float_p, _c_float_p, _c_float_p, ctypes.c_int, ctypes.c_int, ctypes.c_int,
                                                ctypes.c_int, ctypes.c_int, ctypes.c_int, ctypes.c_int, ctypes.c_void_p]),
    "larva_pixel_unshuffle": (ctypes.c_int, [_c_float_p, _c_float_p, ctypes.c_int, ctypes.c_int, ctypes.c_int, ctypes.c_int,
                                             ctypes.c_int, ctypes.c_int, ctypes.c_void_p]),
    "larva_l1_bwd_unshuffle": (ctypes.c_int, [_c_float_p, _c_float_p, _c_float_p, ctypes.c_float, _c_float_p, ctypes.c_int,
                                              ctypes.c_int, ctypes.c_int, ctypes.c_int, ctypes.c_int, ctypes.c_int,
                                              ctypes.c_void_p]),
    "larva_shuffle_l1_partial_grad": (ctypes.c_int, [_c_float_p, _c_float_p, _c_float_p, ctypes.c_float, ctypes.c_float,
                                                     _c_float_p, _c_int_p, _c_float_p, _c_float_p, ctypes.c_int, ctypes.c_int,
                                                     ctypes.c_int, ctypes.c_int, ctypes.c_int, ctypes.c_int, ctypes.c_void_p]),
    "larva_pixel_unshuffle4": (ctypes.c_int, [_c_float_p, _c_float_p, ctypes.c_int, ctypes.c_int,
                                              ctypes.c_int, ctypes.c_int, ctypes.c_void_p]),
    "larva_wgrad_cu_share": (ctypes.c_int, [ctypes.c_int, ctypes.c_int]),
    "larva_adamw_step_host": (ctypes.c_int, [_c_float_p, _c_float_p, _c_float_p, _c_float_p, ctypes.c_int,
                                             ctypes.c_double, ctypes.c_double, ctypes.c_double, ctypes.c_double,
                                             ctypes.c_double, ctypes.c_float, ctypes.c_longlong, ctypes.c_void_p]),
    "larva_gather_patches": (ctypes.c_int, [ctypes.c_void_p, ctypes.c_void_p, ctypes.c_void_p, ctypes.c_void_p,
                                            _c_float_p, ctypes.c_int, ctypes.c_int, ctypes.c_int, ctypes.c_void_p]),
    "larva_sqerr_u8": (ctypes.c_int, [_c_float_p, ctypes.c_void_p, ctypes.c_int, ctypes.c_int, ctypes.c_int,
                                      ctypes.c_int, ctypes.c_int, ctypes.c_void_p, ctypes.c_void_p]),
    "larva_adamw_step": (ctypes.c_int, [_c_float_p, _c_float_p, _c_float_p, _c_float_p, _c_float_p,
                                        ctypes.c_double, ctypes.c_double, ctypes.c_double, ctypes.c_double,
                                        ctypes.c_float, ctypes.c_longlong, ctypes.c_void_p]),
    "larva_f16_packed_weight_halves": (ctypes.c_longlong, [ctypes.c_int, ctypes.c_int]),
    "larva_f16_pack_weights": (ctypes.c_int, [_c_float_p, ctypes.c_void_p, ctypes.c_int, ctypes.c_int, ctypes.c_void_p]),
    "larva_f16_head": (ctypes.c_int, [_c_float_p, _c_float_p, _c_float_p, ctypes.c_void_p, ctypes.c_void_p, ctypes.c_int,
                                      ctypes.c_int, ctypes.c_int, ctypes.c_void_p]),
    "larva_f16_conv3x3": (ctypes.c_int, [_c_pp, ctypes.c_int, ctypes.c_void_p, _c_float_p, ctypes.c_void_p, ctypes.c_void_p,
                                         ctypes.c_int, ctypes.c_void_p, ctypes.c_void_p, ctypes.c_int, ctypes.c_int,
                                         ctypes.c_int, ctypes.c_void_p]),
    "larva_f16_conv3x3_shuffle_base": (ctypes.c_int, [ctypes.c_void_p, ctypes.c_void_p, _c_float_p, _c_float_p, _c_float_p,
                                                      ctypes.c_int, ctypes.c_int, ctypes.c_int, ctypes.c_void_p]),
    "larva_f16_conv3x3_shuffle_base_u8": (ctypes.c_int, [ctypes.c_void_p, ctypes.c_void_p, _c_float_p, _c_float_p,
                                                         ctypes.c_void_p, ctypes.c_void_p, ctypes.c_int, ctypes.c_int,
                                                         ctypes.c_int, ctypes.c_void_p]),
    "larva_f16_conv3x3_jobs": (ctypes.c_int, [ctypes.c_int, _c_pp, _c_pp, _c_pp, ctypes.c_int, _c_pp, ctypes.c_void_p,
                                              ctypes.c_int, ctypes.c_int, ctypes.c_int, ctypes.c_void_p]),
    "larva_f16_conv3x3_shuffle_base_jobs": (ctypes.c_int, [ctypes.c_int, _c_pp, _c_pp, _c_pp, _c_float_p, _c_pp, _c_pp,
                                                           ctypes.c_void_p, ctypes.c_int, ctypes.c_int, ctypes.c_int,
                                                           ctypes.c_void_p]),
    "larva_u8_hwc_to_f32_chw": (ctypes.c_int, [ctypes.c_void_p, _c_float_p, ctypes.c_int, ctypes.c_int, ctypes.c_int,
                                               ctypes.c_void_p]),
    "larva_f32_chw_to_u8_hwc": (ctypes.c_int, [_c_float_p, ctypes.c_void_p, ctypes.c_int, ctypes.c_int, ctypes.c_int,
                                               ctypes.c_void_p]),
    "larva_u8_metrics_workspace_bytes": (ctypes.c_longlong, [ctypes.c_int, ctypes.c_int, ctypes.c_int]),
    "larva_u8_metrics": (ctypes.c_int, [ctypes.c_void_p, ctypes.c_longlong, ctypes.c_void_p, ctypes.c_longlong, ctypes.c_int,
                                        ctypes.c_int, ctypes.c_int, ctypes.c_int, ctypes.c_int, ctypes.c_int,
                                        ctypes.c_void_p, ctypes.c_void_p, ctypes.c_void_p]),
    "larva_dihedral_inputs_u8": (ctypes.c_int, [ctypes.c_void_p, _c_float_p, _c_float_p, ctypes.c_int, ctypes.c_int,
# ... 52 lines not shown
```

### larvanet_amd/kernels.py

```python
import ctypes
import os
import struct

import torch

from . import hip_lib

_SUPPORTED_COUT = (32, 48, 64)


def _stream():
    return torch.cuda.current_stream().cuda_stream


def _chk_tensor(t, name, shape, dtype, last=None):
    if not isinstance(t, torch.Tensor) or not t.is_cuda:
        raise RuntimeError("larvanet_amd: %s must be a tensor on a HIP device (no CPU path exists)" % name)
    kind = str(dtype).replace("torch.", "")
    if last is None:
        if t.dtype != dtype:
            raise RuntimeError("larvanet_amd: %s must be %s, got %s" % (name, kind, t.dtype))
        if not t.is_contiguous():
            raise RuntimeError("larvanet_amd: %s must be contiguous" % name)
    else:
# ... 651 lines not shown
                                              out.data_ptr(), N, C, HH // 4, WW // 4, _stream()),
                  "larva_l1_bwd_unshuffle4")
    return out


def sum_scalars(terms, divisor):
    lib = hip_lib.load()
    ptrs = [_chk(t, "term", ()) for t in terms]
    out = torch.empty((), device=terms[0].device, dtype=torch.float32)
    hip_lib.check(lib.larva_sum_scalars(hip_lib.ptr_array(ptrs), len(ptrs), float(divisor), out.data_ptr(), _stream()),
                  "larva_sum_scalars")
    return out


def l1_bwd(a, b, gout):
    lib = hip_lib.load()
    _chk(a, "a")
    _chk(b, "b", a.shape)
    _chk(gout, "gout", ())
    ga = torch.empty_like(a)
    hip_lib.check(lib.larva_l1_bwd(a.data_ptr(), b.data_ptr(), gout.data_ptr(), a.numel(), ga.data_ptr(), _stream()),
                  "larva_l1_bwd")
    return ga


def pixel_unshuffle4(g):
    lib = hip_lib.load()
    _chk(g, "g")
    N, C, HH, WW = (int(v) for v in g.shape)
    if HH % 4 or WW % 4:
        raise RuntimeError("larvanet_amd: pixel_unshuffle4 needs spatial dims divisible by 4")
    H, W = HH // 4, WW // 4
    out = torch.empty((N, 16 * C, H, W), device=g.device, dtype=torch.float32)
    hip_lib.check(lib.larva_pixel_unshuffle4(g.data_ptr(), out.data_ptr(), N, C, H, W, _stream()),
                  "larva_pixel_unshuffle4")
    return out


def adamw_step(p, g, m, v, step_lr, beta1, beta2, eps, weight_decay, grad_scale=1.0):
    lib = hip_lib.load()
    n = p.numel()
    for t, name in ((p, "p"), (g, "g"), (m, "m"), (v, "v")):
        _chk(t, name, (n,))
    _chk(step_lr, "step_lr", (2,))
    hip_lib.check(lib.larva_adamw_step(p.data_ptr(), g.data_ptr(), m.data_ptr(), v.data_ptr(), step_lr.data_ptr(),
                                       beta1, beta2, eps, weight_decay, grad_scale, n, _stream()),
                  "larva_adamw_step")


def gather_patches(data, offsets, hw, draws, batch, patch, mult, out=None):
    lib = hip_lib.load()
    for t, name, dt in ((data, "data", torch.uint8), (offsets, "offsets", torch.int64), (hw, "hw", torch.int32),
                        (draws, "draws", torch.int32)):
        if not t.is_cuda or t.dtype != dt or not t.is_contiguous():
            raise RuntimeError("larvanet_amd: %s must be a contiguous %s tensor on the HIP device" % (name, dt))
    if tuple(draws.shape) != (batch, 5):
        raise RuntimeError("larvanet_amd: draws must be [batch][5]")
    if out is None:
        out = torch.empty((batch, 3, patch, patch), device=data.device, dtype=torch.float32)
    _chk(out, "out", (batch, 3, patch, patch))
    hip_lib.check(lib.larva_gather_patches(data.data_ptr(), offsets.data_ptr(), hw.data_ptr(), draws.data_ptr(),
                                           out.data_ptr(), batch, patch, mult, _stream()), "larva_gather_patches")
    return out


def adamw_step_host(p, g, m, v, step, lr, beta1, beta2, eps, weight_decay, grad_scale=1.0, copy=None):
    lib = hip_lib.load()
    n = p.numel()
    for t, name in ((p, "p"), (g, "g"), (m, "m"), (v, "v")):
        _chk(t, name, (n,))
    if copy is not None:
        src, dst = copy
        _chk(src, "copy source", ())
        _chk(dst, "copy destination", ())
        hip_lib.check(lib.larva_adamw_step_host_copy(p.data_ptr(), g.data_ptr(), m.data_ptr(), v.data_ptr(), int(step),
                                                     float(lr), beta1, beta2, eps, weight_decay, grad_scale, n,
                                                     src.data_ptr(), dst.data_ptr(), _stream()), "larva_adamw_step_host_copy")
        return
    hip_lib.check(lib.larva_adamw_step_host(p.data_ptr(), g.data_ptr(), m.data_ptr(), v.data_ptr(), int(step),
                                            float(lr), beta1, beta2, eps, weight_decay, grad_scale, n, _stream()),
                  "larva_adamw_step_host")


def psnr_u8(out_chw, truth_u8):
    import math
    lib = hip_lib.load()
    _chk(out_chw, "out")
    if not truth_u8.is_cuda or truth_u8.dtype != torch.uint8 or not truth_u8.is_contiguous():
        raise RuntimeError("larvanet_amd: truth must be a contiguous uint8 tensor on the HIP device")
    C, H, W = (int(v) for v in out_chw.shape)
    TC, TH, TW = (int(v) for v in truth_u8.shape)
    if TC != C or TH < H or TW < W:
        raise RuntimeError("larvanet_amd: truth image smaller than the output")
    acc = torch.zeros(1, device=out_chw.device, dtype=torch.int64)
    hip_lib.check(lib.larva_sqerr_u8(out_chw.data_ptr(), truth_u8.data_ptr(), C, H, W, TH, TW, acc.data_ptr(),
                                     _stream()), "larva_sqerr_u8")
    sq = int(acc.item())
    mse = sq / float(C * H * W)
    return float("inf") if mse == 0 else 10.0 * math.log10(255.0 ** 2 / mse)


F16_CHANNELS = 48
F16_MAX_SOURCES = 8


def _chk16(t, name, shape=None):
    return _chk_tensor(t, name, shape, torch.float16, F16_CHANNELS)


def _chk_wpk16(wpk, n_src, what):
    if wpk.dtype != torch.float16 or not wpk.is_cuda or wpk.numel() != f16_packed_weight_halves(F16_CHANNELS, F16_CHANNELS * n_src):
        raise RuntimeError("larvanet_amd: wpk is not the fp16 image of a %s conv" % what)


def _chk_flag(flag):
    if not isinstance(flag, torch.Tensor) or not flag.is_cuda or flag.dtype != torch.int32 or flag.numel() < 1:
        raise RuntimeError("larvanet_amd: the overflow flag must be an int32 device tensor")
    return flag.data_ptr()


def f16_packed_weight_halves(cout, cin):
    return int(hip_lib.load().larva_f16_packed_weight_halves(cout, cin))


def f16_pack_weights(w, out=None):
    lib = hip_lib.load()
    _chk(w, "w")
    if w.dim() != 4 or tuple(w.shape[2:]) != (3, 3):
        raise RuntimeError("larvanet_amd: only [cout][cin][3][3] weights are supported")
    cout, cin = int(w.shape[0]), int(w.shape[1])
    n = f16_packed_weight_halves(cout, cin)
    if n < 0:
        raise RuntimeError("larvanet_amd: no fp16 conv for %d -> %d channels" % (cin, cout))
    if out is None:
        out = torch.empty(n, device=w.device, dtype=torch.float16)
    if out.dtype != torch.float16 or out.numel() != n or not out.is_contiguous():
        raise RuntimeError("larvanet_amd: fp16 weight image must be %d contiguous halves" % n)
    hip_lib.check(lib.larva_f16_pack_weights(w.data_ptr(), out.data_ptr(), cout, cin, _stream()), "larva_f16_pack_weights")
    return out


def f16_head(x, w, bias, flag, out=None):
    lib = hip_lib.load()
    N, C, H, W = (int(v) for v in x.shape)
    _chk(x, "x")
    _chk(w, "w", (F16_CHANNELS, 3, 3, 3))
    _chk(bias, "bias", (F16_CHANNELS,))
    if C != 3:
        raise RuntimeError("larvanet_amd: the fp16 head takes 3-channel images")
    if out is None:
        out = torch.empty((N, H, W, F16_CHANNELS), device=x.device, dtype=torch.float16)
    _chk16(out, "out", (N, H, W, F16_CHANNELS))
    hip_lib.check(lib.larva_f16_head(x.data_ptr(), w.data_ptr(), bias.data_ptr(), out.data_ptr(), _chk_flag(flag), N, H, W,
                                     _stream()), "larva_f16_head")
    return out


def f16_conv3x3(srcs, wpk, bias, flag, relu=False, res0=None, res1=None, out=None):
    lib = hip_lib.load()
    if isinstance(srcs, torch.Tensor):
        srcs = [srcs]
    if not 1 <= len(srcs) <= F16_MAX_SOURCES:
        raise RuntimeError("larvanet_amd: the fp16 conv takes 1 to %d inputs" % F16_MAX_SOURCES)
    shape = tuple(srcs[0].shape)
    ptrs = [_chk16(s, "srcs[%d]" % i, shape) for i, s in enumerate(srcs)]
    N, H, W = shape[:3]
# ... 322 lines not shown
```

### larvanet_amd/models/LarvaNet.py

```python
import argparse
import copy
import os
import time

import numpy as np
import torch
import torch.nn as nn

from .. import dist as ldist
from .. import kernels as K
from ..autograd import (BodyFn, DeferredWgrad, DualChain, ExitFn, ExitsFn, GradBucket, HeadFn, L1LossFn, LegFn, LossTerm, PackedConv, PaddedWidth, mean_of_terms,
                        StepScope, is_large_inference, pack_all)
from ..autograd import step_prologue as autograd_step_prologue
from ..captured_step import CapturedStep, LossCopy
from ..infer_graphs import Form, GraphTable
from ..optim import FlatAdamW, flatten_parameters
from ..metrics import image_psnr, image_to_uint8, fit_truth_image_size
from .base import BaseModel

SUPPORTED_INTERPOLATE = ("bicubic", "bilinear")

NUM_FILTERS = 48
SUPPORTED_NUM_FILTERS = (32, 48, 64)
SCALED_COUT_PAD = 32
# ... 84 lines not shown

    merges = False

    def forward(self, fea, base):
        _require_hip(fea)
        return run_leg(self, fea, base)


def run_leg(end, fea, base, truth=None, divisor=None):
    for pc in end._pcs:
        pc.refresh()
    if end.merges:
        fea = end.merge(fea)
    c1, c2 = end.recon_block[0], end.recon_block[2]
    params = (c1.weight, c1.bias, c2.weight, c2.bias)
    if truth is None:
        return LegFn.apply(fea.contiguous(), base.contiguous(), end._pcs, end.scale, *params)
    return ExitFn.apply(fea.contiguous(), base.contiguous(), truth.contiguous(), end._pcs, end.scale, divisor, *params)


class LarvaBody(nn.Module):

    def __init__(self, num_blocks, num_filters=NUM_FILTERS, scale=4):
        super().__init__()
        self.res_blocks = nn.Sequential(*[ResidualBlock(num_filters) for _ in range(num_blocks)])
        self.leg = LarvaLeg(num_filters, scale)
        self._pcs = []
        for blk in self.res_blocks:
            self._pcs += [PackedConv(blk.body[0].weight, blk.body[0].bias),
                          PackedConv(blk.body[2].weight, blk.body[2].bias)]

    def forward(self, x):
        _require_hip(x)
        params = []
        for blk in self.res_blocks:
            params += [blk.body[0].weight, blk.body[0].bias, blk.body[2].weight, blk.body[2].bias]
        if not params:
            return x + x
        for pc in self._pcs:
            pc.refresh()
        return BodyFn.apply(x.contiguous(), self._pcs, *params)


def parse_num_blocks(args):
    blocks = [int(v) for v in str(args.num_blocks).split(",")]
    if len(blocks) != args.num_modules:
        raise GeneratorExit("Argument num_blocks should have the same number of elements as num_modules.")
    return blocks


class LarvaNetModule(nn.Module):

    def __init__(self, args):
        super().__init__()
        self.len = args.num_modules
        self.interpolate = args.interpolate
        self.pad_odd_widths = True
        self.num_filters = int(getattr(args, "num_filters", NUM_FILTERS))
        if self.num_filters not in SUPPORTED_NUM_FILTERS:
            raise ValueError("larvanet_amd: --num_filters must be one of %s" % (SUPPORTED_NUM_FILTERS,))
        self.scale = int(getattr(args, "scale", 4))
        self._half = None
        self.head = LarvaHead(self.num_filters)
        for i, nb in enumerate(parse_num_blocks(args)):
            setattr(self, "body_%d" % i, LarvaBody(num_blocks=nb, num_filters=self.num_filters, scale=self.scale))
        self._join_input_grads()

    def _join_input_grads(self):
        from ..autograd import JointBwd
        for i in range(self.len - 1):
            nxt = getattr(self, "body_%d" % (i + 1))
            if nxt._pcs:
                JointBwd(nxt._pcs[0], getattr(self, "body_%d" % i).leg._pcs[0])

    def packed_convs(self):
        out = []
        for m in self.modules():
            out += ([m._pc] if hasattr(m, "_pc") else []) + list(getattr(m, "_pcs", []))
        return out

    def invalidate_packed_weights(self):
        for pc in self.packed_convs():
            pc.invalidate()
        if self._half is not None:
            self._half.invalidate()

    def half_forward(self):
        if self._half is None:
            from ..half import HalfForward
            self._half = HalfForward(self)
        return self._half

    def refresh_packed_weights(self):
        pack_all(self.packed_convs())

    def step_prologue(self, x):
        _require_hip(x)
        res = autograd_step_prologue(self.packed_convs(), x) if self.interpolate == "bicubic" and self.scale == 4 else None
        if res is None:
            self.refresh_packed_weights()
            return self.base(x), None
        return res[1], res[0]

    def base(self, x):
        _require_hip(x)
        if self.interpolate not in SUPPORTED_INTERPOLATE:
            raise ValueError("larvanet_amd: --interpolate=%s has no HIP kernel; supported: %s"
                             % (self.interpolate, ", ".join(SUPPORTED_INTERPOLATE)))
        with torch.no_grad():
            return K.upsample(x.detach().contiguous(), self.scale, self.interpolate)

    def width_scope(self, x):
        w = int(x.shape[-1])
        if w % 4 and self.pad_odd_widths and not (torch.is_grad_enabled() and any(p.requires_grad for p in self.parameters())):
            return PaddedWidth(w)
        return _NoScope()

    def bodies(self, n):
        return [getattr(self, "body_%d" % i) for i in range(n)]

    def route(self):
        return self.len, getattr(self, "body_%d" % (self.len - 1)).leg

    def exit_route(self):
        bodies, end = self.route()
        name = type(self).__module__.rsplit(".", 1)[-1]
        if end is not None and end.merges:
            raise ValueError("larvanet_amd: %s has no per-body exits: its route ends in a tail that merges every body's "
                             "output (all-exit inference is for LarvaNet / LarvaLeg)" % name)
        if not bodies:
            raise ValueError("larvanet_amd: %s --leg=0 returns the base image alone: there is no exit to list" % name)
        return bodies, [body.leg for body in self.bodies(bodies)]

    def forward_exits(self, x, batched=True):
        bodies, legs = self.exit_route()
        base = self.base(x)
        with self.width_scope(x):
            fea = self.head(x)
            feas = []
            for body in self.bodies(bodies):
                fea = body(fea)
                feas.append(fea)
            DualChain.join()
            M = len(legs)
            out = torch.empty((M,) + tuple(base.shape), device=base.device, dtype=torch.float32)
            if not (batched and self.scale == 4 and M > 1):
                for i, leg in enumerate(legs):
                    out[i].copy_(leg(feas[i], base))
                return out
            for leg in legs:
                for pc in leg._pcs:
                    pc.refresh()
            lw = PaddedWidth.current
            i = 0
            while i < M:
                n = 3 if M - i == 5 else min(4, M - i)
                c1 = [leg.recon_block[0] for leg in legs[i:i + n]]
                c2 = [leg.recon_block[2] for leg in legs[i:i + n]]
                hs = K.conv3x3_batch([{"srcs": feas[i + k].contiguous(), "wpk": legs[i + k]._pcs[0].get()[0][0],
                                       "bias": c1[k].bias.detach()} for k in range(n)],
                                     int(c1[0].weight.shape[0]), relu=True, logical_w=lw)
                K.conv3x3_batch([{"srcs": hs[k], "wpk": legs[i + k]._pcs[1].get()[0][0], "bias": c2[k].bias.detach(),
                                  "base": base} for k in range(n)],
                                int(c2[0].weight.shape[0]), shuffle=True, logical_w=lw, outs=[out[i + k] for k in range(n)])
                i += n
            return out

    def forward(self, x):
        bodies, end = self.route()
        base = self.base(x)
        if end is None:
            return base
        with self.width_scope(x):
            fea = self.head(x)
            feats = []
            for body in self.bodies(bodies):
                fea = body(fea)
                if end.merges:
                    feats.append(fea)
            DualChain.join()
            return end(feats if end.merges else fea, base)


class LarvaNet(BaseModel):

    module_class = LarvaNetModule

    def __init__(self):
        super().__init__()
        self.volume_per_step = 0
        self.sync_loss = True
        self.early_loss = {"0": False, "split": "split"}.get(os.environ.get("LARVA_EARLY_LOSS", "poll"), "poll")
        self.use_hip_graph = os.environ.get("LARVA_HIP_GRAPH", "1") != "0"
        self.hip_graph_fell_back = None
        self.strict_graph = os.environ.get("LARVA_HIP_GRAPH_STRICT", "0") != "0"
        self.defer_wgrad = os.environ.get("LARVA_DEFER_WGRAD", "1") != "0"
        self.joint_input_grads = os.environ.get("LARVA_JOINT_DGRAD", "1") != "0"
        self.batch_exits = os.environ.get("LARVA_BATCH_EXITS", "1") != "0"
        self.overlap_allreduce = {"0": False, "1": True}.get(os.environ.get("LARVA_OVERLAP_ALLREDUCE", "auto"), "auto")
        self.dp_schedule = None
        self.dual_chain = os.environ.get("LARVA_DUAL_CHAIN", "1") != "0"
        self.force_split_backward = os.environ.get("LARVA_FORCE_SPLIT", "0") != "0"
        self.args = None
        self.precision = "fp32"
        self.grad_bucket = None
        self.time_allreduce = False
        self.allreduce_events = []
        self._step = None
        self._infer_graphs, self._infer_graphs_u8, self._infer_graphs_se = GraphTable(), GraphTable(), GraphTable()
        self._infer_graphs_ex = GraphTable()
        self.batch_exit_legs = None
        self._one = self._late = self._early_lo = None
        self._loss_in_flight = False
        self._handoffs = {}

    has_cooldown = True

    def _add_args(self, parser):
        parser.add_argument("--num_modules", type=int, default=2, help="Number of cascaded bodies (exits).")
        parser.add_argument("--num_blocks", type=str, default="16,16", help="Residual blocks per body, comma separated.")
        parser.add_argument("--interpolate", type=str, default="bicubic", help="Interpolation of the base image.")
        parser.add_argument("--val_volume", type=float, default=30e9, help="Input volume between validations.")
        parser.add_argument("--lr", type=float, default=4e-4, help="Initial learning rate.")
        parser.add_argument("--lr_decay", type=float, default=0.5, help="Learning rate decay factor.")
        parser.add_argument("--lr_step", type=int, default=20000, help="Learning rate decay step (unused, kept for CLI parity).")
        parser.add_argument("--threshold", type=float, default=0.001, help="Plateau threshold (absolute, dB).")
        parser.add_argument("--min_lr", type=float, default=1e-8, help="Minimum learning rate.")
        parser.add_argument("--patience", type=int, default=3, help="Plateau patience.")
        parser.add_argument("--cooldown", type=int, default=6, help="Plateau cooldown.")
        self._add_build_args(parser)

    def _add_build_args(self, parser):
        parser.add_argument("--num_filters", type=int, default=NUM_FILTERS, choices=SUPPORTED_NUM_FILTERS,
                            help="Channels of the head / bodies / legs (the legs' last conv keeps 48). "
                                 "The reference hard-wires 48.")
        parser.add_argument("--precision", type=str, default="fp32", choices=SUPPORTED_PRECISIONS,
                            help="Activation precision of inference (upscale / test / fwd_runtime): fp16 stores "
                                 "activations in fp16 and accumulates in fp32 (x4, --num_filters 48 only). "
                                 "Training is always fp32.")
        parser.add_argument("--self_ensemble", action="store_true",
                            help="Geometric self-ensemble (x8) in upscale / upscale_u8 / evaluate_u8_tensor and the "
                                 "streams: the mean of the image's eight flips and transposes run through the network "
                                 "and mapped back, merged on the device.")

    def parse_args(self, args):
        parser = argparse.ArgumentParser()
        self._add_args(parser)
        self.args, remaining_args = parser.parse_known_args(args=args)
        if self.args.interpolate not in SUPPORTED_INTERPOLATE:
            raise ValueError("larvanet_amd: --interpolate=%s has no HIP kernel; supported: %s"
                             % (self.args.interpolate, ", ".join(SUPPORTED_INTERPOLATE)))
        return copy.deepcopy(self.args), remaining_args

    def _make_scheduler(self):
        return torch.optim.lr_scheduler.ReduceLROnPlateau(
            self.optim, mode="max", factor=self.args.lr_decay, patience=self.args.patience,
            cooldown=self.args.cooldown if self.has_cooldown else 0,
            threshold=self.args.threshold, threshold_mode="abs", min_lr=self.args.min_lr)

    def prepare(self, is_training, scales, global_step=0):
        self.global_step = global_step
        self.total_volume = 0.0
        self.temp_volume = 0
        self.scale_list = scales
        for scale in self.scale_list:
            if scale not in (2, 3, 4):
                raise ValueError("Unsupported scale is provided.")
        if len(self.scale_list) != 1:
            raise ValueError("Only one scale should be provided.")
        self.scale = self.scale_list[0]
        nf = int(getattr(self.args, "num_filters", NUM_FILTERS))
        if self.scale != 4 and nf != NUM_FILTERS:
            raise ValueError("larvanet_amd: --num_filters %d at x%d is not supported (x2 / x3 networks are built at "
                             "--num_filters %d only)" % (nf, self.scale, NUM_FILTERS))
        self.precision = getattr(self.args, "precision", "fp32")
        if self.precision not in SUPPORTED_PRECISIONS:
            raise ValueError("larvanet_amd: --precision must be one of %s" % (SUPPORTED_PRECISIONS,))
        if self.precision == "fp16" and (self.scale != 4 or nf != NUM_FILTERS):
            raise ValueError("larvanet_amd: --precision fp16 is built for x4 at --num_filters %d only (got x%d, "
                             "--num_filters %d)" % (NUM_FILTERS, self.scale, nf))
        if self.precision == "fp16" and min(parse_num_blocks(self.args)) < 1:
            raise ValueError("larvanet_amd: --precision fp16 needs at least one residual block per body")

        self.device = torch.device("cuda", torch.cuda.current_device()) if torch.cuda.is_available() \
            else torch.device("cpu")
        self._step = self._one = self._late = self._early_lo = self.grad_bucket = None
        self._loss_in_flight = False
        for table in (self._infer_graphs, self._infer_graphs_u8, self._infer_graphs_se, self._infer_graphs_ex):
            table.clear()
        margs = copy.copy(self.args)
        margs.scale = self.scale
        self.model = self.module_class(args=margs).to(self.device)
        ldist.broadcast_parameters(self.model)

        if is_training:
            self.loss_fn = L1Loss()
            params = [p for p in self.model.parameters() if p.requires_grad]
            if self.device.type == "cuda":
                flat = flatten_parameters(self.model)
                self.model.invalidate_packed_weights()
                self.grad_bucket = GradBucket(self.model, self.model.packed_convs())
                self.optim = FlatAdamW(params, flat, self.grad_bucket, lr=self.args.lr)
                self._choose_dp_schedule()
            else:
                self.optim = torch.optim.AdamW(params, lr=self.args.lr)
                if self.overlap_allreduce == "auto":
                    self.overlap_allreduce = False
                self.dp_schedule = {"choice": "flat", "why": "CPU tensors: one collective over flattened gradients"}
            self.scheduler = self._make_scheduler()

    DP_SPLIT_ABOVE_US = 90.0

    def _choose_dp_schedule(self):
        ws = ldist.world_size()
        if self.overlap_allreduce != "auto":
            self.overlap_allreduce = bool(self.overlap_allreduce)
            self.dp_schedule = {"why": "LARVA_OVERLAP_ALLREDUCE"}
        elif not ldist.active():
            self.overlap_allreduce = True
            self.dp_schedule = {"why": "one rank, no communicator"}
        else:
            t_us = ldist.time_allreduce_us(self.grad_bucket.flat)
            self.overlap_allreduce = t_us > self.DP_SPLIT_ABOVE_US
            self.dp_schedule = {"allreduce_isolated_us": t_us, "bucket_bytes": int(self.grad_bucket.flat.numel()) * 4, "ranks": ws,
                                "rule": "split (two weight-gradient launch groups, the first slice all-reduced beside the second) "
                                        "when the isolated all-reduce of the bucket takes more than %.0f us" % self.DP_SPLIT_ABOVE_US}
        self.dp_schedule["choice"] = "split" if self._split_backward() else "flat"
        if self.force_split_backward:
            self.dp_schedule["forced"] = "LARVA_FORCE_SPLIT"
        if ldist.active() and ldist.is_main() and "allreduce_isolated_us" in self.dp_schedule:
            print("data-parallel weight-gradient schedule: %s (isolated all-reduce of the %.2f MB bucket over %d ranks: %.1f us)"
                  % (self.dp_schedule["choice"], self.dp_schedule["bucket_bytes"] / 1e6, ws, self.dp_schedule["allreduce_isolated_us"]))

    def _grad_one(self, loss):
        if self._one is None or self._one.device != loss.device:
            self._one = torch.ones((), device=loss.device, dtype=loss.dtype)
        return self._one

    def _num_loss_terms(self):
        return self.args.num_modules

    def _exit(self, leg, fea, base, truth_tensor):
        if isinstance(self.loss_fn, L1Loss) and isinstance(leg, LarvaLeg):
            out, part = run_leg(leg, fea, base, truth_tensor, self._num_loss_terms())
            return out, LossTerm(part, 1.0 / float(out.numel()), prescaled=True)
        out = leg(fea, base)
        return out, self.loss_fn(out, truth_tensor)

    def _exits_batched(self):
        return (self.batch_exits and isinstance(self.loss_fn, L1Loss) and PaddedWidth.current is None
                and self.model.scale == 4
                and all(isinstance(getattr(self.model, "body_%d" % i).leg, LarvaLeg) for i in range(self.args.num_modules)))

    def _all_exits(self, feas, base, truth_tensor):
        legs, params = [], []
        for i in range(len(feas)):
            leg = getattr(self.model, "body_%d" % i).leg
            for pc in leg._pcs:
                pc.refresh()
            legs.append(leg._pcs)
            c1, c2 = leg.recon_block[0], leg.recon_block[2]
            params += [c1.weight, c1.bias, c2.weight, c2.bias]
        res = ExitsFn.apply(base.contiguous(), truth_tensor.contiguous(), legs, self._num_loss_terms(),
                            *[f.contiguous() for f in feas], *params)
        scale = 1.0 / float(res[0].numel())
        return res[0], [LossTerm(p, scale, prescaled=True) for p in res[1:]]

    def _exit_losses(self, input_tensor, truth_tensor):
        net = self.model
        base, x16 = net.step_prologue(input_tensor)
        fea = net.head(input_tensor, x16)
        if self._exits_batched():
            feas = []
            for i in range(self.args.num_modules):
                fea = getattr(net, "body_%d" % i)(fea)
                feas.append(fea)
            DualChain.join()
            out, terms = self._all_exits(feas, base, truth_tensor)
            return mean_of_terms(terms), out
        terms = []
        out = None
        for i in range(self.args.num_modules):
            body = getattr(net, "body_%d" % i)
            fea = body(fea)
            out, term = self._exit(body.leg, fea, base, truth_tensor)
            terms.append(term)
        return mean_of_terms(terms), out

    def _graph_key(self, input_tensor, truth_tensor):
        mode = ("split" if self.early_loss == "split" else "poll") if self.sync_loss and self.early_loss else False
        return (tuple(input_tensor.shape), tuple(truth_tensor.shape), str(input_tensor.device), mode)

    def _scope(self, early_loss=False):
        lazy_fwd = self._exits_batched()
        lazy_bwd = (lazy_fwd and self.joint_input_grads and self.defer_wgrad and self._single_consumer_features()
                    and self.grad_bucket is not None and self.grad_bucket.intact(self.model))
        return StepScope(defer_wgrad=self.defer_wgrad, split_flush=self._split_backward(),
                         joint_input_grads=self.joint_input_grads, seed_grad=1.0, dual_chain=self.dual_chain,
                         lazy_chain_joins=(lazy_fwd, lazy_bwd), early_loss=early_loss)

    def _single_consumer_features(self):
        return True

    def _split_backward(self):
        return (self.overlap_allreduce is True and self.defer_wgrad and (ldist.active() or self.force_split_backward)
                and self.grad_bucket is not None and self.grad_bucket.intact(self.model))

    def _step_body(self, input_tensor, truth_tensor, early_loss=False, cut=None):
        with self._scope(early_loss=early_loss) as scope:
            loss, out = self._exit_losses(input_tensor, truth_tensor)
            if cut is not None:
                cut()
            loss.backward(self._grad_one(loss))
        bucket, early_lo = self.grad_bucket, None
        if scope.split_flush and bucket is not None and scope.early_targets:
            early, late = bucket.span(scope.early_targets), bucket.span(DeferredWgrad.late_targets())
            if early is not None and late is not None and early[1] == bucket.flat.numel() and late[1] <= early[0]:
                early_lo = early[0]
        return loss, out, early_lo

    _graph_late = property(lambda self: self._step and self._step.late)

    def input_buffers(self, input_shape, truth_shape):
        if not self.use_hip_graph or self._step is None:
            return None
        return self._step.buffers(input_shape, truth_shape)

    def _zero_grad(self):
        bucket = self.grad_bucket
        if bucket is not None and bucket.intact(self.model):
            return
        if bucket is not None:
            for pc in self.model.packed_convs():
                pc.grad_inplace = False
            self.grad_bucket = None
        self.optim.zero_grad(set_to_none=True)

    def _forward_backward(self, input_tensor, truth_tensor):
        if self.use_hip_graph and input_tensor.is_cuda:
            key = self._graph_key(input_tensor, truth_tensor)
            if self._step is None or self._step.key != key:
                try:
                    mode = key[-1]
                    if mode and mode not in self._handoffs:
                        self._handoffs[mode] = K.HostCell() if mode == "poll" else LossCopy()
                    self._step = CapturedStep(self, key, mode, self._handoffs.get(mode), input_tensor, truth_tensor)
                except Exception as e:
                    if self.strict_graph:
                        raise
                    print("WARNING: hipGraph capture failed (%s: %s); continuing with eager launches"
                          % (type(e).__name__, e))
                    self.use_hip_graph = False
                    self.hip_graph_fell_back = "%s: %s" % (type(e).__name__, e)
                    torch.cuda.synchronize()
                    DualChain.reset()
                    return self._forward_backward(input_tensor, truth_tensor)
            step = self._step
            step.stage(input_tensor, truth_tensor)
            self._loss_in_flight, self._early_lo = step.mode, step.early_lo
            loss, out, self._late = step.replay()
            return loss, out
        self._zero_grad()
        loss, out, self._early_lo = self._step_body(input_tensor, truth_tensor)
        self._late = DeferredWgrad.flush_late if DeferredWgrad.has_late() else None
        return loss, out

    def _finish_backward(self):
        late, self._late = self._late, None
        ws = ldist.world_size()
        bucket = self.grad_bucket
        if not ldist.active() or bucket is None or not bucket.intact(self.model):
            if late is not None:
                late()
            ldist.allreduce_gradients(self.model, None)
            if isinstance(self.optim, FlatAdamW):
                self.optim.mean_scale = 1.0
            return
        lo = self._early_lo
        timed = self.time_allreduce and self.device.type == "cuda"
        if late is None or lo is None or lo <= 0:
            if late is not None:
                late()
            t0 = self._mark(timed)
            ldist.allreduce_sum(bucket.flat)
        else:
            work = ldist.allreduce_sum(bucket.flat[lo:], async_op=True)
            late()
            t0 = self._mark(timed)
            ldist.allreduce_sum(bucket.flat[:lo])
            work.wait()
        if timed:
            self.allreduce_events.append((t0, self._mark(True)))
        if isinstance(self.optim, FlatAdamW):
            self.optim.mean_scale = 1.0 / ws
        else:
            bucket.flat.mul_(1.0 / ws)

    def _mark(self, on):
        if not on:
            return None
        ev = torch.cuda.Event(enable_timing=True)
        ev.record()
        return ev

    def train_step_larva(self, args, val_dataloader, input_tensor, truth_tensor, summary=None):
        n, c, h, w = (int(v) for v in input_tensor.shape)
        s = self.model.scale
        if tuple(truth_tensor.shape) != (n, c, s * h, s * w):
            raise ValueError("larvanet_amd: truth of shape %s for an input of %s at x%d; expected %s"
                             % (tuple(truth_tensor.shape), tuple(input_tensor.shape), s, (n, c, s * h, s * w)))
        self.global_step += 1
        self.temp_volume += self.volume_per_step

        loss, out = self._forward_backward(input_tensor, truth_tensor)
        self._finish_backward()
        loss_copy = None
        if not self.sync_loss and isinstance(self.optim, FlatAdamW) and loss.is_cuda:
            loss_copy = torch.empty_like(loss)
            self.optim.copy_scalar = (loss.detach(), loss_copy)
        self.optim.step()
        if loss_copy is not None and self.optim.copy_scalar is not None:
            self.optim.copy_scalar = None
            loss_copy = None
        self.model.invalidate_packed_weights()

        if self.global_step == 1:
            self.validate_for_train(args, val_dataloader)

        if self.temp_volume >= self.args.val_volume:
            self.total_volume += self.temp_volume
            self.temp_volume = 0
            self.validate_for_train(args, val_dataloader)
            if ldist.is_main():
                self.save(base_path=args.train_path)
                if getattr(args, "save_train_state", False):
                    self.save_training_state(base_path=args.train_path)
                print(f"saved a model checkpoint at volume {self.total_volume/1e9:.0f}G")
            if summary is not None:
                self._write_summary(summary, loss, input_tensor, out, truth_tensor)

        if self.sync_loss:
            how, self._loss_in_flight = self._loss_in_flight, False
            if how == "split":
                return self._handoffs["split"].result()
            if how == "poll":
                return self._poll_loss()
            return loss.item()
        self._loss_in_flight = False
        return loss_copy if loss_copy is not None else loss.detach().clone()

    def _poll_loss(self):
        cell = self._handoffs["poll"]
        t0 = time.perf_counter()
        spins = 0
        while True:
            v = cell.take()
            if v is not None:
                return v
            spins += 1
            if spins > 2000:
                dt = time.perf_counter() - t0
                if dt > 5.0:
                    break
                time.sleep(0 if dt < 0.02 else 0.0005)
        torch.cuda.current_stream().synchronize()
        v = cell.take()
        if v is None:
            raise RuntimeError("larvanet_amd: the captured step finished without storing its loss "
                               "(host cell at sequence %d, expected %d)" % (cell.sequence, cell.expected))
        return v

    def _write_summary(self, summary, loss, input_tensor, out, truth_tensor):
        summary.add_scalar("loss", loss, self.global_step)
        summary.add_scalar("lr", self.get_lr(), self.global_step)
        tensors = {"input": input_tensor, "output": out.detach(), "truth": truth_tensor}
        for name, t in tensors.items():
            t8 = t.clamp(0, 255).byte()
            for i in range(min(4, len(t8))):
                summary.add_image("%s/%d" % (name, i), t8[i], self.global_step)

    def validate_for_train(self, args, dataloader):
        print("begin validation")
        num_images = dataloader.get_num_images()
        psnr_sum = 0.0
        with torch.no_grad():
            for image_index in range(ldist.rank(), num_images, ldist.world_size()):
                input_image, truth_image, _ = dataloader.get_image_pair(image_index=image_index, scale=self.scale)
                psnr_sum += self.image_psnr(input_image, truth_image)
        average_psnr = ldist.allreduce_scalar_sum(psnr_sum, self.device) / max(num_images, 1)
        print(f"step {self.global_step}, volume {self.total_volume/1e9:.0f}G,"
              f" psnr={average_psnr:.8f}, lr = {self.get_lr():.8f}")
        self.scheduler.step(average_psnr)
        return average_psnr

    def image_psnr(self, input_image, truth_image):
        if self.device.type == "cuda":
            out = self.model(self._to_input_tensor([input_image]))[0].contiguous()
            truth8 = torch.from_numpy(np.ascontiguousarray(image_to_uint8(truth_image))).to(self.device)
            return K.psnr_u8(out, truth8)
        output_image = image_to_uint8(self.upscale(input_list=[input_image], scale=self.scale)[0])
        truth8 = fit_truth_image_size(output_image=output_image, truth_image=image_to_uint8(truth_image))
        return float(image_psnr(output_image=output_image, truth_image=truth8))

    def _infer_scope(self):
        return StepScope(defer_wgrad=False, joint_input_grads=False, dual_chain=self.dual_chain,
                         lazy_chain_joins=(True, False))

    def _eager_or_graph(self, x, form):
        n = int(x.shape[0])
        h, w = (int(v) for v in (x.shape[1:3] if form.u8 else x.shape[2:4]))
        if not (self.use_hip_graph and x.is_cuda) or is_large_inference((8 if h == w else 4) * n if form.ensemble else n, h, w):
            return self._forward_nograd(x, *form, exits=form.exits)
        table = (self._infer_graphs_ex if form.exits else self._infer_graphs_se if form.ensemble
                 else self._infer_graphs_u8 if form.u8 else self._infer_graphs)
        tag = ("u8" if form.u8 else "f32", "se") if form.ensemble else ("u8",) if form.u8 else ()
        return table.forward((tuple(x.shape), self.precision) + tag, x, capture=lambda x: self._capture_infer(x, form),
                             run=lambda x: self._forward_nograd(x, *form, exits=form.exits))

    def _infer(self, x):
        return self.model(x) if torch.is_grad_enabled() else self._eager_or_graph(x, Form())

    def _infer_u8(self, x_u8):
        return self._eager_or_graph(x_u8, Form(u8=True))

    def _infer_ensemble(self, x, u8=False):
        return self._eager_or_graph(x, Form(u8, True))

    def _infer_u8_images(self, x_u8):
        return self._eager_or_graph(x_u8, Form(True, self._self_ensemble()))

    def _capture_infer(self, x, form):
        static_x = x.clone()
# ... 272 lines not shown
```

### larvanet_amd/optim.py

```python
import torch

from . import kernels as K


def flatten_parameters(module):
    params = [p for p in module.parameters() if p.requires_grad]
    flat = torch.empty(sum(p.numel() for p in params), device=params[0].device, dtype=torch.float32)
    off = 0
    with torch.no_grad():
        for p in params:
            view = flat[off:off + p.numel()].view_as(p)
            view.copy_(p.data)
            p.data = view
            off += p.numel()
    return flat


class FlatAdamW(torch.optim.AdamW):
    def __init__(self, params, flat_params, grad_bucket, lr=1e-3, **kw):
        params = list(params)
        super().__init__(params, lr=lr, **kw)
        self._flat_p = flat_params
        self._bucket = grad_bucket
        self._m = torch.zeros_like(flat_params)
        self._v = torch.zeros_like(flat_params)
        self._t = 0
        self._plist = params
        self.copy_scalar = None
        self.mean_scale = 1.0

    def _flat_ok(self):
        if self._flat_p is None or self._bucket is None or not self._bucket.intact():
            return False
        off = 0
        base = self._flat_p.data_ptr()
        for p in self._plist:
            if p.data_ptr() != base + 4 * off:
                return False
            off += p.numel()
        return True

    @torch.no_grad()
    def step(self, closure=None):
        if closure is not None or len(self.param_groups) != 1 or not self._flat_ok():
            return self._fallback_step(closure)
        g = self.param_groups[0]
        if g.get("amsgrad") or g.get("maximize"):
            return self._fallback_step(closure)
        self._t += 1
        b1, b2 = g["betas"]
        copy, self.copy_scalar = self.copy_scalar, None
        K.adamw_step_host(self._flat_p, self._bucket.flat, self._m, self._v, self._t, float(g["lr"]), b1, b2,
                          g["eps"], g["weight_decay"], self.mean_scale, copy=copy)
        return None

    def training_state(self):
        if self._flat_p is not None:
            return {"flat": True, "t": self._t, "m": self._m.detach().cpu().clone(), "v": self._v.detach().cpu().clone(),
                    "param_groups": [{k: v for k, v in g.items() if k != "params"} for g in self.param_groups]}
        return {"flat": False, "torch": super().state_dict()}

    def load_training_state(self, st):
        if st.get("flat") and self._flat_p is not None:
            self._t = int(st["t"])
            self._m.copy_(st["m"].to(self._m.device))
            self._v.copy_(st["v"].to(self._v.device))
            for g, saved in zip(self.param_groups, st["param_groups"]):
                g.update(saved)
        elif not st.get("flat"):
            super().load_state_dict(st["torch"])
        else:
            raise RuntimeError("larvanet_amd: flat optimizer state cannot be loaded into a per-tensor optimizer")

    def _fallback_step(self, closure):
        if self.mean_scale != 1.0:
            for p in self._plist:
                if p.grad is not None:
                    p.grad.mul_(self.mean_scale)
            self.mean_scale = 1.0
        if self._t > 0 and not self.state:
            off = 0
            for p in self._plist:
                n = p.numel()
                self.state[p] = {"step": torch.tensor(float(self._t)),
                                 "exp_avg": self._m[off:off + n].view_as(p).clone(),
                                 "exp_avg_sq": self._v[off:off + n].view_as(p).clone()}
                off += n
        self._flat_p = None
        return super().step(closure)
```

Before: 362.9 HR Mpixels/s.

## Fuse wgrad reduction, AdamW update and weight repacking into one finishing launch

The final weight-gradient reduction is held back past backward and replaced by one kernel that reduces the partials, applies AdamW per element, and writes the packed forward and backward weight images directly. The next step's prologue then skips weight packing. This removes the separate optimizer launch, the repack pass, and a round trip over gradients and parameters. In exchange it adds bookkeeping for when the fused path applies, with fallbacks to the old path, and a more complex reduction kernel that may have lower occupancy.

```diff
diff --git a/include/larva_hip.h b/include/larva_hip.h
--- a/include/larva_hip.h
+++ b/include/larva_hip.h
@@ -89,6 +89,14 @@
                                  const int* splits, const int* cout, const int* cin, int njobs,
                                  const float* const* terms, const int* count, const float* scale, int nterms,
                                  float divisor, float* loss_out, void* stream);
+
+int larva_wgrad_reduce_finish(const float* const* partial, float* const* dw, float* const* db, const int* cin_off,
+                              const int* cin_valid, const int* w_cin_total, const int* splits, const int* cout,
+                              const int* cin, int njobs, float* const* wpk_fwd, float* const* wpk_bwd, const float* g,
+                              float* p, float* m, float* v, long long n, const float* step_lr, int step, double lr,
+                              double beta1, double beta2, double eps, double weight_decay, float grad_scale,
+                              const float* const* terms, const int* count, const float* scale, int nterms,
+                              float divisor, float* loss_out, const float* copy_src, float* copy_dst, void* stream);
 
 int larva_bicubic4_fwd(const float* in, float* out, int N, int C, int H, int W, void* stream);
 int larva_upsample4_fwd(const float* in, float* out, int N, int C, int H, int W, int mode, void* stream);
diff --git a/larvanet_amd/autograd.py b/larvanet_amd/autograd.py
--- a/larvanet_amd/autograd.py
+++ b/larvanet_amd/autograd.py
@@ -116,7 +116,7 @@
 class PackedConv:
 
     __slots__ = ("weight", "bias", "cin_pad", "slices", "_key", "_packs", "_bufs", "_prepacked", "grad_inplace",
-                 "joint", "joint_slot", "cout_pad", "_pad")
+                 "joint", "joint_slot", "cout_pad", "_pad", "flat")
 
     def __init__(self, weight, bias, cin_pad=None, slices=None, cout_pad=None):
         self.weight, self.bias, self.cin_pad = weight, bias, cin_pad
@@ -128,6 +128,7 @@
         self._packs = None
         self._bufs = None
         self._prepacked = False
+        self.flat = None
         self.joint = None
         self.joint_slot = 0
 
@@ -137,7 +138,7 @@
 
     def _current_key(self):
         w = self.weight
-        return (w.data_ptr(), w._version, str(w.device))
+        return (w.data_ptr(), w._version, str(w.device), None if self.flat is None else self.flat._version)
 
     def jobs(self):
         w = self.weight
@@ -243,9 +244,9 @@
         return hit[0]
 
 
-def step_prologue(pcs, x):
+def step_prologue(pcs, x, pack=True):
     jobs = []
-    for pc in pcs:
+    for pc in pcs if pack else ():
         jobs += pc.jobs()
     N, C, H, W = (int(v) for v in x.shape)
     if len(jobs) > 64 or C > 16 or PaddedWidth.current is not None or not x.is_contiguous():
@@ -255,7 +256,8 @@
     with torch.no_grad():
         K.step_prologue(jobs, x.detach(), x16, base)
     for pc in pcs:
-        pc._mark_packed()
+        if pack:
+            pc._mark_packed()
         pc._prepacked = True
     return x16, base
 
@@ -313,6 +315,39 @@
     return max(1, _WGRAD_WORKGROUPS * K.wgrad_cu_share(cout, cin) // njobs)
 
 
+class HeldReduce:
+
+    def __init__(self, jobs, loss):
+        self.jobs, self.loss = jobs, loss
+        self._finish = None
+
+    def reduce_only(self):
+        K.wgrad_reduce(self.jobs, loss=self.loss)
+
+    def finisher(self, pcs, g, p, m, v):
+        key = (g.data_ptr(), p.data_ptr(), m.data_ptr(), v.data_ptr())
+        if self._finish is not None and self._finish[0] == key:
+            return self._finish[1]
+        images = {}
+        for pc in pcs:
+            if pc.slices is not None or pc.cout_pad is not None or not pc.grad_inplace or pc.weight.grad is None:
+                return None
+            (_, fwd, bwd, cout, cin_k, _), = pc.jobs()
+            images[pc.weight.grad.data_ptr()] = (fwd, bwd, cout, cin_k)
+        jobs, covered = [], 0
+        for j in self.jobs:
+            hit = images.pop(j["dw"].data_ptr(), None)
+            if hit is None or j.get("db") is None or j.get("cin_off", 0) or (hit[2], hit[3]) != (j["cout"], j["cin"]):
+                return None
+            jobs.append(dict(j, wpk_fwd=hit[0], wpk_bwd=hit[1]))
+            covered += j["dw"].numel() + j["db"].numel()
+        launch = None
+        if not images and covered == p.numel() and len(jobs) <= K.WgradReduceFinish.MAX_JOBS:
+            launch = K.WgradReduceFinish(jobs, g, p, m, v, loss=self.loss)
+        self._finish = (key, launch)
+        return launch
+
+
 class DeferredWgrad:
 
     active = False
@@ -345,8 +380,11 @@
             terms, scales, divisor, out = job
             out.copy_(K.loss_from_partials(terms, scales, divisor))
 
-    @staticmethod
-    def _issue(launches):
+    hold = False
+    held = None
+
+    @staticmethod
+    def _issue(launches, hold=False):
         reduce_jobs = []
         head = host = None
         heads = [l for l in launches if (l[0], l[1]) == (48, 16) and len(l[2]) == 1]
@@ -368,6 +406,9 @@
                 continue
             parts, used = K.conv3x3_wgrad_partial(chunk, cout, cin, _splits(len(chunk), cout, cin))
             reduce_jobs += [dict(j, partial=p, splits=used, cout=cout, cin=cin) for j, p in zip(chunk, parts)]
+        if hold and 1 <= len(reduce_jobs) <= K.WgradReduceFinish.MAX_JOBS:
+            DeferredWgrad.held, DeferredWgrad.pending_loss = HeldReduce(reduce_jobs, DeferredWgrad.pending_loss), None
+            return
         for i in range(0, len(reduce_jobs), 64):
             last = i + 64 >= len(reduce_jobs)
             loss, DeferredWgrad.pending_loss = (DeferredWgrad.pending_loss, None) if last else (None, DeferredWgrad.pending_loss)
@@ -377,7 +418,7 @@
     def flush(cls, split=False):
         launches = cls._launches(split)
         n_early = max(1, len(launches) // 2) if split else len(launches)
-        cls._issue(launches[:n_early])
+        cls._issue(launches[:n_early], hold=cls.hold and not split)
         cls._late = launches[n_early:]
         if not split:
             return None
@@ -401,6 +442,7 @@
         cls._pending = {}
         cls._late = []
         cls.pending_loss = None
+        cls.held = None
 
 
 class StepScope:
@@ -421,8 +463,10 @@
         return buf
 
     def __init__(self, defer_wgrad=True, split_flush=False, joint_input_grads=True,
-                 seed_grad=None, dual_chain=False, lazy_chain_joins=(False, False), early_loss=False):
+                 seed_grad=None, dual_chain=False, lazy_chain_joins=(False, False), early_loss=False, hold_reduce=False):
         self.seed_grad_value = seed_grad
+        self.hold_reduce = bool(hold_reduce) and not split_flush
+        self.held = None
         self.early_loss_value = early_loss or False
         self.dual_chain = dual_chain
         self.lazy_chain_joins = lazy_chain_joins
@@ -435,6 +479,7 @@
         gpu = torch.cuda.is_available()
         DeferredWgrad.active = bool(self.defer_wgrad) and gpu
         DeferredWgrad.drop()
+        DeferredWgrad.hold = self.hold_reduce and DeferredWgrad.active
         JointInputGrad.active = bool(self.joint_input_grads) and gpu
         JointInputGrad.reset()
         DualChain.enabled = bool(self.dual_chain) and gpu
@@ -449,6 +494,7 @@
             DualChain.join()
             if exc_type is None:
                 self.early_targets = DeferredWgrad.flush(split=self.split_flush)
+                self.held, DeferredWgrad.held = DeferredWgrad.held, None
                 DeferredWgrad.finish_loss()
             else:
                 DeferredWgrad.drop()
@@ -461,7 +507,7 @@
             StepScope.early_loss = False
             DeferredWgrad._pending = {}
             DualChain.enabled = DualChain.lazy_fwd = DualChain.lazy_bwd = False
-            DeferredWgrad.active = False
+            DeferredWgrad.active = DeferredWgrad.hold = False
             JointInputGrad.active = False
             JointInputGrad.reset()
         return False
diff --git a/larvanet_amd/build.py b/larvanet_amd/build.py
--- a/larvanet_amd/build.py
+++ b/larvanet_amd/build.py
@@ -7,7 +7,7 @@
 LIB = os.path.join(CSRC, "liblarva_hip.so")
 SOURCES = ["conv3x3_mfma.hip", "wgrad3x3_mfma.hip", "larva_pointwise.hip", "larva_scale.hip", "conv3x3_f16.hip",
            "larva_metrics.hip", "larva_ensemble.hip", "larva_downscale.hip"]
-HEADERS = ["larva_common.h", "larva_bicubic.h", "larva_loss.h"]
+HEADERS = ["larva_common.h", "larva_bicubic.h", "larva_loss.h", "larva_adamw.h"]
 FLAGS = ["--offload-arch=gfx950", "-O3", "-std=c++17", "-fPIC", "-Wall", "-Wno-unused-function"]
 
 
diff --git a/larvanet_amd/captured_step.py b/larvanet_amd/captured_step.py
--- a/larvanet_amd/captured_step.py
+++ b/larvanet_amd/captured_step.py
@@ -57,6 +57,7 @@
         self.static_in, self.static_truth = x, truth
         self.graph, self.back, self.late = graph, back, late
         self.loss, self.out, self.early_lo = loss, out, early_lo
+        self.held = plugin._held
 
     def stage(self, input_tensor, truth_tensor):
         for dst, src in ((self.static_in, input_tensor), (self.static_truth, truth_tensor)):
diff --git a/larvanet_amd/csrc/conv3x3_mfma.hip b/larvanet_amd/csrc/conv3x3_mfma.hip
--- a/larvanet_amd/csrc/conv3x3_mfma.hip
+++ b/larvanet_amd/csrc/conv3x3_mfma.hip
@@ -953,7 +953,6 @@
   const int cols = fwd ? j.cout : j.cin;
   const int cs = cout_stride(cols);
   const int tid = threadIdx.x;
-  out += (size_t)chunk * 72 * cs;
   for (int c0 = 0; c0 < cs; c0 += kPackTileCols) {
     const int ncol = min(kPackTileCols, cols - c0);
     if (fwd) {
@@ -974,11 +973,9 @@
     }
     __syncthreads();
     const int wcols = min(kPackTileCols, cs - c0);
-    const bool swz = cout_swizzled(cols);
     for (int idx = tid; idx < 72 * wcols; idx += 256) {
       const int r = idx / wcols, c = idx - r * wcols;
-      const int col = swz ? ((c0 + c) ^ ((r & 1) << 4)) : c0 + c;
-      out[r * cs + col] = c < ncol ? tile[r * kPackLd + c] : 0.f;
+      out[packed_weight_index(cols, chunk, r, c0 + c)] = c < ncol ? tile[r * kPackLd + c] : 0.f;
     }
     __syncthreads();
   }
diff --git a/larvanet_amd/csrc/larva_adamw.h b/larvanet_amd/csrc/larva_adamw.h
--- /dev/null
+++ b/larvanet_amd/csrc/larva_adamw.h
@@ -0,0 +1,42 @@
+#pragma once
+#include "larva_common.h"
+
+namespace larva {
+
+struct AdamwCoef {
+  float step_size, bc2_sqrt, decay;
+};
+
+__device__ __forceinline__ AdamwCoef adamw_coef_device(float step, float lr, double beta1, double beta2, float wd) {
+  const double bc1 = 1.0 - pow(beta1, (double)step);
+  const double bc2 = 1.0 - pow(beta2, (double)step);
+  return AdamwCoef{(float)((double)lr / bc1), (float)sqrt(bc2), (float)(1.0 - (double)lr * (double)wd)};
+}
+
+inline AdamwCoef adamw_coef_host(int step, double lr, double beta1, double beta2, double wd) {
+  const double bc1 = 1.0 - pow(beta1, (double)step), bc2 = 1.0 - pow(beta2, (double)step);
+  return AdamwCoef{(float)(lr / bc1), (float)sqrt(bc2), (float)(1.0 - lr * wd)};
+}
+
+__device__ __forceinline__ float rounded(float x) {
+  asm volatile("" : "+v"(x));
+  return x;
+}
+
+struct AdamwBetas {
+  float beta2, omb1, omb2;
+};
+
+__host__ __device__ inline AdamwBetas adamw_betas(double beta1, double beta2) {
+  return AdamwBetas{(float)beta2, (float)(1.0 - beta1), (float)(1.0 - beta2)};
+}
+
+__device__ __forceinline__ void adamw_update(float& param, float& mi, float& vi, float grad, const AdamwCoef& c,
+                                             const AdamwBetas& b, float eps) {
+  mi = __fmaf_rn(b.omb1, rounded(grad - mi), mi);
+  vi = __fmaf_rn(rounded(b.omb2 * grad), grad, rounded(vi * b.beta2));
+  const float denom = rounded(__fdiv_rn(__fsqrt_rn(vi), c.bc2_sqrt)) + eps;
+  param = rounded(param * c.decay) + rounded(__fdiv_rn(rounded(-c.step_size * mi), denom));
+}
+
+}
diff --git a/larvanet_amd/csrc/larva_common.h b/larvanet_amd/csrc/larva_common.h
--- a/larvanet_amd/csrc/larva_common.h
+++ b/larvanet_amd/csrc/larva_common.h
@@ -45,6 +45,10 @@
   return (cout % 32 == 16 || cout % 32 == 0) ? cout : cout + 16;
 }
 __host__ __device__ constexpr bool cout_swizzled(int cout) { return cout % 32 == 0; }
+
+__host__ __device__ constexpr int packed_weight_index(int cols, int chunk, int r, int c) {
+  return (chunk * 72 + r) * cout_stride(cols) + (cout_swizzled(cols) ? (c ^ ((r & 1) << 4)) : c);
+}
 
 __device__ __forceinline__ int xcd_remap(int b, int nwg) {
   const int q = nwg >> 3, r = nwg & 7, xcd = b & 7;
diff --git a/larvanet_amd/csrc/larva_pointwise.hip b/larvanet_amd/csrc/larva_pointwise.hip
--- a/larvanet_amd/csrc/larva_pointwise.hip
+++ b/larvanet_amd/csrc/larva_pointwise.hip
@@ -1,6 +1,7 @@
 #include "larva_common.h"
 #include "larva_bicubic.h"
 #include "larva_loss.h"
+#include "larva_adamw.h"
 
 namespace larva {
 
@@ -412,32 +413,6 @@
   }
 }
 
-struct AdamwCoef {
-  float step_size, bc2_sqrt, decay;
-};
-
-__device__ __forceinline__ AdamwCoef adamw_coef_device(float step, float lr, double beta1, double beta2, float wd) {
-  const double bc1 = 1.0 - pow(beta1, (double)step);
-  const double bc2 = 1.0 - pow(beta2, (double)step);
-  return AdamwCoef{(float)((double)lr / bc1), (float)sqrt(bc2), (float)(1.0 - (double)lr * (double)wd)};
-}
-
-__device__ __forceinline__ float rounded(float x) {
-  asm volatile("" : "+v"(x));
-  return x;
-}
-
-struct AdamwBetas {
-  float beta2, omb1, omb2;
-};
-
-__device__ __forceinline__ void adamw_update(float& param, float& mi, float& vi, float grad, const AdamwCoef& c,
-                                             const AdamwBetas& b, float eps) {
-  mi = __fmaf_rn(b.omb1, rounded(grad - mi), mi);
-  vi = __fmaf_rn(rounded(b.omb2 * grad), grad, rounded(vi * b.beta2));
-  const float denom = rounded(__fdiv_rn(__fsqrt_rn(vi), c.bc2_sqrt)) + eps;
-  param = rounded(param * c.decay) + rounded(__fdiv_rn(rounded(-c.step_size * mi), denom));
-}
 
 __global__ __launch_bounds__(256) void adamw_kernel(float* __restrict__ p, const float* __restrict__ g,
                                                     float* __restrict__ m, float* __restrict__ v,
@@ -800,8 +775,7 @@
                                double beta2, double eps, double weight_decay, float grad_scale, long long n,
                                const float* copy_src, float* copy_dst, void* stream) {
   if (!p || !g || !m || !v || n <= 0 || step < 1 || (copy_dst && !copy_src)) return (int)hipErrorInvalidValue;
-  const double bc1 = 1.0 - pow(beta1, (double)step), bc2 = 1.0 - pow(beta2, (double)step);
-  const AdamwCoef coef{(float)(lr / bc1), (float)sqrt(bc2), (float)(1.0 - lr * weight_decay)};
+  const AdamwCoef coef = adamw_coef_host(step, lr, beta1, beta2, weight_decay);
   hipLaunchKernelGGL(adamw_kernel, dim3(grid_for((n + 3) / 4, 256)), dim3(256), 0, (hipStream_t)stream, p, g, m, v,
                      (const float*)nullptr, coef, beta1, beta2, (float)eps, (float)weight_decay, grad_scale, n, adamw_vec_ok(p, g, m, v),
                      copy_src, copy_dst);
diff --git a/larvanet_amd/csrc/wgrad3x3_mfma.hip b/larvanet_amd/csrc/wgrad3x3_mfma.hip
--- a/larvanet_amd/csrc/wgrad3x3_mfma.hip
+++ b/larvanet_amd/csrc/wgrad3x3_mfma.hip
@@ -1,5 +1,6 @@
 #include "larva_common.h"
 #include "larva_loss.h"
+#include "larva_adamw.h"
 
 #include <type_traits>
 
@@ -900,6 +901,7 @@
 };
 
 constexpr int kMaxReduceJobs = 64;
+constexpr int kMaxFinishJobs = 48;
 
 struct ReduceBatch {
   ReduceJob job[kMaxReduceJobs];
@@ -954,20 +956,56 @@
   }
 }
 
-__global__ __launch_bounds__(256) void wgrad_reduce_kernel(ReduceBatch rb) {
-  if ((int)blockIdx.y == rb.njobs) {
-    if (blockIdx.x == 0) loss_terms_block(rb.loss_terms, rb.loss_divisor, rb.loss_out);
-    return;
-  }
-  __shared__ float tile[16 * kReduceRow];
+struct StepFinish {
+  float* fwd[kMaxFinishJobs];
+  float* bwd[kMaxFinishJobs];
+  const float* g;
+  float* p;
+  float* m;
+  float* v;
+  const float* step_lr;
+  AdamwCoef coef;
+  double beta1, beta2;
+  float eps, wd, gscale;
+  const float* copy_src;
+  float* copy_dst;
+};
+
+struct FinishBatch {
+  ReduceJob job[kMaxFinishJobs];
+  int njobs;
+  TermList loss_terms;
+  float loss_divisor;
+  float* loss_out;
+  StepFinish fin;
+};
+
+__device__ __forceinline__ float finish_element(const StepFinish& f, const AdamwCoef& coef, const AdamwBetas& bt,
+                                                size_t off, float grad) {
+  float pp = f.p[off], mm = f.m[off], vv = f.v[off];
+  adamw_update(pp, mm, vv, __fmul_rn(grad, f.gscale), coef, bt, f.eps);
+  f.p[off] = pp; f.m[off] = mm; f.v[off] = vv;
+  return pp;
+}
+
+template <bool FINISH, typename Batch>
+__device__ __forceinline__ void reduce_block(const Batch& rb, const StepFinish* fin, float* tile) {
   const ReduceJob& j = rb.job[blockIdx.y];
-  if (j.splits > kReduceColumnwiseAbove) return reduce_columnwise(j);
+  if constexpr (!FINISH) {
+    if (j.splits > kReduceColumnwiseAbove) return reduce_columnwise(j);
+  }
   const int ct_n = j.cout / 16;
   const int c = blockIdx.x % ct_n, cit = blockIdx.x / ct_n;
   if (cit >= j.cin / 16) return;
   const int n_w = (j.cin / 16) * 9 * ct_n * 256;
   const int pf = n_w + j.cout;
   const int tid = threadIdx.x;
+  AdamwCoef coef{};
+  AdamwBetas bt{};
+  if constexpr (FINISH) {
+    coef = fin->step_lr ? adamw_coef_device(fin->step_lr[0], fin->step_lr[1], fin->beta1, fin->beta2, fin->wd) : fin->coef;
+    bt = adamw_betas(fin->beta1, fin->beta2);
+  }
   if (tid < 192) {
     const int lane = tid & 63, tap0 = tid >> 6;
     f32x4 s[3];
@@ -1002,15 +1040,63 @@
     float sb = 0.f;
     for (int k = 0; k < j.splits; ++k) sb += p[(size_t)k * pf];
     j.db[c * 16 + (tid - 192)] = sb;
+    if constexpr (FINISH) finish_element(*fin, coef, bt, (size_t)(j.db + c * 16 + (tid - 192) - fin->g), sb);
   }
   __syncthreads();
   const int ci_n = min(16, j.cin_valid - cit * 16);
 #pragma unroll
   for (int e = 0; e < 9; ++e) {
     const int idx = e * 256 + tid, co = idx / 144, rem = idx - co * 144;
-    if (rem < ci_n * 9)
-      j.dw[((size_t)(c * 16 + co) * j.w_cin_total + j.cin_off + cit * 16) * 9 + rem] = tile[co * kReduceRow + rem];
-  }
+    if (rem < ci_n * 9) {
+      float* dst = j.dw + ((size_t)(c * 16 + co) * j.w_cin_total + j.cin_off + cit * 16) * 9 + rem;
+      const float g = tile[co * kReduceRow + rem];
+      *dst = g;
+      if constexpr (FINISH) tile[co * kReduceRow + rem] = finish_element(*fin, coef, bt, (size_t)(dst - fin->g), g);
+    } else if constexpr (FINISH) {
+      tile[co * kReduceRow + rem] = 0.f;
+    }
+  }
+  if constexpr (FINISH) {
+    __syncthreads();
+    float* __restrict__ fwd = fin->fwd[blockIdx.y];
+    float* __restrict__ bwd = fin->bwd[blockIdx.y];
+#pragma unroll
+    for (int e = 0; e < 9; ++e) {
+      const int idx = e * 256 + tid, co = idx & 15, row = idx >> 4, ci = row / 9, tap = row - ci * 9;
+      const int cl = cit * 16 + ci;
+      fwd[packed_weight_index(j.cout, cl >> 3, tap * 8 + (cl & 7), c * 16 + co)] = tile[co * kReduceRow + ci * 9 + tap];
+    }
+    if (bwd) {
+#pragma unroll
+      for (int e = 0; e < 9; ++e) {
+        const int idx = e * 256 + tid, ci = idx & 15, row = idx >> 4, co = row / 9, tap = row - co * 9;
+        const int ca = c * 16 + co;
+        bwd[packed_weight_index(j.cin, ca >> 3, (8 - tap) * 8 + (ca & 7), cit * 16 + ci)] = tile[co * kReduceRow + ci * 9 + tap];
+      }
+    }
+  }
+}
+
+__global__ __launch_bounds__(256) void wgrad_reduce_kernel(ReduceBatch rb) {
+  if ((int)blockIdx.y == rb.njobs) {
+    if (blockIdx.x == 0) loss_terms_block(rb.loss_terms, rb.loss_divisor, rb.loss_out);
+    return;
+  }
+  __shared__ float tile[16 * kReduceRow];
+  reduce_block<false>(rb, nullptr, tile);
+}
+
+__global__ __launch_bounds__(256) void wgrad_reduce_finish_kernel(FinishBatch rb) {
+  if ((int)blockIdx.y == rb.njobs) {
+    if (blockIdx.x == 0) {
+      if (rb.loss_terms.n) loss_terms_block(rb.loss_terms, rb.loss_divisor, rb.loss_out);
+      __syncthreads();
+      if (rb.fin.copy_dst && threadIdx.x == 0) rb.fin.copy_dst[0] = *(const volatile float*)rb.fin.copy_src;
+    }
+    return;
+  }
+  __shared__ float tile[16 * kReduceRow];
+  reduce_block<true>(rb, &rb.fin, tile);
 }
 
 template <int COUT, int CIN>
@@ -1284,6 +1370,55 @@
                        stream);
 }
 
+int larva_wgrad_reduce_finish(const float* const* partial, float* const* dw, float* const* db, const int* cin_off,
+                              const int* cin_valid, const int* w_cin_total, const int* splits, const int* cout,
+                              const int* cin, int njobs, float* const* wpk_fwd, float* const* wpk_bwd, const float* g,
+                              float* p, float* m, float* v, long long n, const float* step_lr, int step, double lr,
+                              double beta1, double beta2, double eps, double weight_decay, float grad_scale,
+                              const float* const* terms, const int* count, const float* scale, int nterms,
+                              float divisor, float* loss_out, const float* copy_src, float* copy_dst, void* stream) {
+  if (njobs < 1 || njobs > kMaxFinishJobs || !wpk_fwd || !wpk_bwd || !g || !p || !m || !v || n <= 0) return (int)hipErrorInvalidValue;
+  if ((!step_lr && step < 1) || nterms < 0 || nterms > 8 || (copy_dst && !copy_src)) return (int)hipErrorInvalidValue;
+  if (nterms && (!terms || !count || !scale || !loss_out)) return (int)hipErrorInvalidValue;
+  FinishBatch rb{};
+  int pf_max = 0;
+  for (int i = 0; i < njobs; ++i) {
+    if (!partial[i] || !dw[i] || !wpk_fwd[i] || splits[i] < 1 || cout[i] <= 0 || cin[i] <= 0 || cout[i] % 16 || cin[i] % 16 ||
+        cin_off[i] < 0 || cin_valid[i] < 1 || cin_valid[i] > cin[i] || cin_off[i] + cin_valid[i] > w_cin_total[i])
+      return (int)hipErrorInvalidValue;
+    if (splits[i] > kReduceColumnwiseAbove) return (int)hipErrorNotSupported;
+    const long long wo = dw[i] - g, wn = (long long)cout[i] * w_cin_total[i] * 9;
+    if (dw[i] < g || wo + wn > n) return (int)hipErrorInvalidValue;
+    if (db && db[i] && (db[i] < g || (db[i] - g) + cout[i] > n)) return (int)hipErrorInvalidValue;
+    rb.job[i] = ReduceJob{partial[i], dw[i], db ? db[i] : nullptr, cin_off[i], cin_valid[i], w_cin_total[i],
+                          splits[i], cout[i], cin[i]};
+    rb.fin.fwd[i] = wpk_fwd[i];
+    rb.fin.bwd[i] = wpk_bwd[i];
+    const int pf = (cout[i] / 16) * (cin[i] / 16);
+    pf_max = pf > pf_max ? pf : pf_max;
+  }
+  rb.njobs = njobs;
+  for (int i = 0; i < nterms; ++i) {
+    if (!terms[i] || count[i] < 1) return (int)hipErrorInvalidValue;
+    rb.loss_terms.p[i] = terms[i];
+    rb.loss_terms.count[i] = count[i];
+    rb.loss_terms.scale[i] = scale[i];
+  }
+  rb.loss_terms.n = nterms;
+  rb.loss_divisor = divisor;
+  rb.loss_out = loss_out;
+  StepFinish& f = rb.fin;
+  f.g = g; f.p = p; f.m = m; f.v = v;
+  f.step_lr = step_lr;
+  if (!step_lr) f.coef = adamw_coef_host(step, lr, beta1, beta2, weight_decay);
+  f.beta1 = beta1; f.beta2 = beta2;
+  f.eps = (float)eps; f.wd = (float)weight_decay; f.gscale = grad_scale;
+  f.copy_src = copy_src; f.copy_dst = copy_dst;
+  hipLaunchKernelGGL(wgrad_reduce_finish_kernel, dim3(pf_max, njobs + ((nterms || copy_dst) ? 1 : 0)), dim3(256), 0,
+                     (hipStream_t)stream, rb);
+  return (int)hipGetLastError();
+}
+
 int larva_conv3x3_wgrad(const float* const* dy, const float* const* x, float* const* partial,
                         float* const* dw, float* const* db, const int* cin_off,
                         const int* cin_valid, const int* w_cin_total, int njobs, int splits,
diff --git a/larvanet_amd/hip_lib.py b/larvanet_amd/hip_lib.py
--- a/larvanet_amd/hip_lib.py
+++ b/larvanet_amd/hip_lib.py
@@ -67,6 +67,12 @@
     "larva_wgrad_reduce_with_loss": (ctypes.c_int, [_c_pp, _c_pp, _c_pp, _c_int_p, _c_int_p, _c_int_p, _c_int_p, _c_int_p,
                                                     _c_int_p, ctypes.c_int, _c_pp, _c_int_p, _c_float_p, ctypes.c_int,
                                                     ctypes.c_float, _c_float_p, ctypes.c_void_p]),
+    "larva_wgrad_reduce_finish": (ctypes.c_int, [_c_pp, _c_pp, _c_pp, _c_int_p, _c_int_p, _c_int_p, _c_int_p, _c_int_p,
+                                                 _c_int_p, ctypes.c_int, _c_pp, _c_pp, _c_float_p, _c_float_p, _c_float_p,
+                                                 _c_float_p, ctypes.c_longlong, _c_float_p, ctypes.c_int, ctypes.c_double,
+                                                 ctypes.c_double, ctypes.c_double, ctypes.c_double, ctypes.c_double,
+                                                 ctypes.c_float, _c_pp, _c_int_p, _c_float_p, ctypes.c_int, ctypes.c_float,
+                                                 _c_float_p, _c_float_p, _c_float_p, ctypes.c_void_p]),
     "larva_adamw_step_host_copy": (ctypes.c_int, [_c_float_p, _c_float_p, _c_float_p, _c_float_p, ctypes.c_int,
                                                   ctypes.c_double, ctypes.c_double, ctypes.c_double, ctypes.c_double,
                                                   ctypes.c_double, ctypes.c_float, ctypes.c_longlong, _c_float_p, _c_float_p,
diff --git a/larvanet_amd/kernels.py b/larvanet_amd/kernels.py
--- a/larvanet_amd/kernels.py
+++ b/larvanet_amd/kernels.py
@@ -757,6 +757,61 @@
                   "larva_adamw_step_host")
 
 
+class WgradReduceFinish:
+
+    MAX_JOBS = 48
+
+    def __init__(self, jobs, g, p, m, v, loss=None):
+        if not 1 <= len(jobs) <= self.MAX_JOBS:
+            raise RuntimeError("larvanet_amd: 1..%d reduce jobs per finishing launch" % self.MAX_JOBS)
+        n = int(p.numel())
+        for t, name in ((p, "p"), (g, "g"), (m, "m"), (v, "v")):
+            _chk(t, name, (n,))
+        parts, dws, dbs, offs, valids, totals, splits, couts, cins, fwds, bwds = ([] for _ in range(11))
+        for j in jobs:
+            co, ci = int(j["cout"]), int(j["cin"])
+            dw = j["dw"]
+            _chk(dw, "dw")
+            if dw.dim() != 4 or int(dw.shape[0]) != co or tuple(dw.shape[2:]) != (3, 3):
+                raise RuntimeError("larvanet_amd: dw must be [cout][cin_total][3][3]")
+            total, off, valid = int(dw.shape[1]), int(j.get("cin_off", 0)), int(j.get("cin_valid", ci))
+            if off < 0 or valid < 1 or valid > ci or off + valid > total:
+                raise RuntimeError("larvanet_amd: wgrad channel slice out of range")
+            sp = int(j["splits"])
+            parts.append(_chk(j["partial"], "partial", (wgrad_partial_floats(co, ci, sp),)))
+            dws.append(dw.data_ptr())
+            dbs.append(_opt(j.get("db"), "db", (co,)))
+            fwds.append(_chk(j["wpk_fwd"], "wpk_fwd", (packed_weight_floats(co, ci),)))
+            bwds.append(_opt(j.get("wpk_bwd"), "wpk_bwd", (packed_weight_floats(ci, co),)))
+            for lst, val in ((offs, off), (valids, valid), (totals, total), (splits, sp), (couts, co), (cins, ci)):
+                lst.append(val)
+        self._head = (hip_lib.ptr_array(parts), hip_lib.ptr_array(dws), hip_lib.ptr_array(dbs), hip_lib.int_array(offs),
+                      hip_lib.int_array(valids), hip_lib.int_array(totals), hip_lib.int_array(splits),
+                      hip_lib.int_array(couts), hip_lib.int_array(cins), len(jobs), hip_lib.ptr_array(fwds),
+                      hip_lib.ptr_array(bwds), g.data_ptr(), p.data_ptr(), m.data_ptr(), v.data_ptr(), n)
+        if loss is None:
+            self._loss = (None, None, None, 0, 1.0, None)
+        else:
+            terms, scales, divisor, out = loss
+            if not 1 <= len(terms) <= 8:
+                raise RuntimeError("larvanet_amd: 1..8 loss terms")
+            _chk(out, "loss", ())
+            self._loss = _loss_terms(terms, scales) + (len(terms), float(divisor), out.data_ptr())
+        self._keep = (jobs, g, p, m, v, loss)
+
+    def launch(self, step, lr, beta1, beta2, eps, weight_decay, grad_scale=1.0, copy=None, step_lr=None):
+        src = dst = None
+        if copy is not None:
+            src, dst = (_chk(copy[0], "copy source", ()), _chk(copy[1], "copy destination", ()))
+        sl = None if step_lr is None else _chk(step_lr, "step_lr", (2,))
+        code = hip_lib.load().larva_wgrad_reduce_finish(*self._head, sl, int(step), float(lr), beta1, beta2, eps,
+                                                        weight_decay, grad_scale, *self._loss, src, dst, _stream())
+        if code == 801:
+            return False
+        hip_lib.check(code, "larva_wgrad_reduce_finish")
+        return True
+
+
 def psnr_u8(out_chw, truth_u8):
     import math
     lib = hip_lib.load()
diff --git a/larvanet_amd/models/LarvaNet.py b/larvanet_amd/models/LarvaNet.py
--- a/larvanet_amd/models/LarvaNet.py
+++ b/larvanet_amd/models/LarvaNet.py
@@ -190,6 +190,9 @@
     def invalidate_packed_weights(self):
         for pc in self.packed_convs():
             pc.invalidate()
+        self.invalidate_half_weights()
+
+    def invalidate_half_weights(self):
         if self._half is not None:
             self._half.invalidate()
 
@@ -202,11 +205,15 @@
     def refresh_packed_weights(self):
         pack_all(self.packed_convs())
 
-    def step_prologue(self, x):
+    def packed_weights_stale(self):
+        return any(pc._packs is None or pc._key != pc._current_key() for pc in self.packed_convs())
+
+    def step_prologue(self, x, pack=True):
         _require_hip(x)
-        res = autograd_step_prologue(self.packed_convs(), x) if self.interpolate == "bicubic" and self.scale == 4 else None
+        res = autograd_step_prologue(self.packed_convs(), x, pack=pack) if self.interpolate == "bicubic" and self.scale == 4 else None
         if res is None:
-            self.refresh_packed_weights()
+            if pack:
+                self.refresh_packed_weights()
             return self.base(x), None
         return res[1], res[0]
 
@@ -319,6 +326,10 @@
         self._infer_graphs_ex = GraphTable()
         self.batch_exit_legs = None
         self._one = self._late = self._early_lo = None
+        self.finish_in_reduction = False
+        self._hold = False
+        self._held = None
+        self._packed_at = None
         self._loss_in_flight = False
         self._handoffs = {}
 
@@ -393,6 +404,7 @@
         self.device = torch.device("cuda", torch.cuda.current_device()) if torch.cuda.is_available() \
             else torch.device("cpu")
         self._step = self._one = self._late = self._early_lo = self.grad_bucket = None
+        self.finish_in_reduction, self._hold, self._held, self._packed_at = False, False, None, None
         self._loss_in_flight = False
         for table in (self._infer_graphs, self._infer_graphs_u8, self._infer_graphs_se, self._infer_graphs_ex):
             table.clear()
@@ -406,10 +418,13 @@
             params = [p for p in self.model.parameters() if p.requires_grad]
             if self.device.type == "cuda":
                 flat = flatten_parameters(self.model)
+                for pc in self.model.packed_convs():
+                    pc.flat = flat
                 self.model.invalidate_packed_weights()
                 self.grad_bucket = GradBucket(self.model, self.model.packed_convs())
                 self.optim = FlatAdamW(params, flat, self.grad_bucket, lr=self.args.lr)
                 self._choose_dp_schedule()
+                self._choose_step_finish()
             else:
                 self.optim = torch.optim.AdamW(params, lr=self.args.lr)
                 if self.overlap_allreduce == "auto":
@@ -440,6 +455,24 @@
             print("data-parallel weight-gradient schedule: %s (isolated all-reduce of the %.2f MB bucket over %d ranks: %.1f us)"
                   % (self.dp_schedule["choice"], self.dp_schedule["bucket_bytes"] / 1e6, ws, self.dp_schedule["allreduce_isolated_us"]))
 
+    def _choose_step_finish(self):
+        pcs = self.model.packed_convs()
+        owned = {id(t) for pc in pcs for t in (pc.weight, pc.bias)}
+        why = None
+        if ldist.active():
+            why = "data parallel: an all-reduce stands between reduction and update"
+        elif self._split_backward():
+            why = "split weight-gradient schedule"
+        elif not self.defer_wgrad:
+            why = "weight gradients are not deferred"
+        elif any(pc.slices is not None or pc.cout_pad is not None or not pc.grad_inplace for pc in pcs):
+            why = "a conv over concatenated inputs or padded outputs"
+        elif any(id(p) not in owned for p in self.model.parameters() if p.requires_grad):
+            why = "a parameter that is no conv's weight or bias"
+        self.finish_in_reduction = why is None
+        self.dp_schedule["step_finish"] = "one launch: reduction + AdamW + packed weights" if why is None \
+            else "reduction, optimizer launch, repack in the next prologue (%s)" % why
+
     def _grad_one(self, loss):
         if self._one is None or self._one.device != loss.device:
             self._one = torch.ones((), device=loss.device, dtype=loss.dtype)
@@ -476,7 +509,7 @@
 
     def _exit_losses(self, input_tensor, truth_tensor):
         net = self.model
-        base, x16 = net.step_prologue(input_tensor)
+        base, x16 = net.step_prologue(input_tensor, pack=not self._hold)
         fea = net.head(input_tensor, x16)
         if self._exits_batched():
             feas = []
@@ -497,7 +530,7 @@
 
     def _graph_key(self, input_tensor, truth_tensor):
         mode = ("split" if self.early_loss == "split" else "poll") if self.sync_loss and self.early_loss else False
-        return (tuple(input_tensor.shape), tuple(truth_tensor.shape), str(input_tensor.device), mode)
+        return (tuple(input_tensor.shape), tuple(truth_tensor.shape), str(input_tensor.device), self._hold, mode)
 
     def _scope(self, early_loss=False):
         lazy_fwd = self._exits_batched()
@@ -505,7 +538,7 @@
                     and self.grad_bucket is not None and self.grad_bucket.intact(self.model))
         return StepScope(defer_wgrad=self.defer_wgrad, split_flush=self._split_backward(),
                          joint_input_grads=self.joint_input_grads, seed_grad=1.0, dual_chain=self.dual_chain,
-                         lazy_chain_joins=(lazy_fwd, lazy_bwd), early_loss=early_loss)
+                         lazy_chain_joins=(lazy_fwd, lazy_bwd), early_loss=early_loss, hold_reduce=self._hold)
 
     def _single_consumer_features(self):
         return True
@@ -520,6 +553,7 @@
             if cut is not None:
                 cut()
             loss.backward(self._grad_one(loss))
+        self._held = scope.held
         bucket, early_lo = self.grad_bucket, None
         if scope.split_flush and bucket is not None and scope.early_targets:
             early, late = bucket.span(scope.early_targets), bucket.span(DeferredWgrad.late_targets())
@@ -567,6 +601,7 @@
             step.stage(input_tensor, truth_tensor)
             self._loss_in_flight, self._early_lo = step.mode, step.early_lo
             loss, out, self._late = step.replay()
+            self._held = step.held
             return loss, out
         self._zero_grad()
         loss, out, self._early_lo = self._step_body(input_tensor, truth_tensor)
@@ -620,17 +655,34 @@
         self.global_step += 1
         self.temp_volume += self.volume_per_step
 
-        loss, out = self._forward_backward(input_tensor, truth_tensor)
+        self._hold = self._finish_applies(input_tensor)
+        try:
+            if self._hold and self._packed_images_stale():
+                self.model.refresh_packed_weights()
+                self._packed_at = self.optim.flat_version()
+            loss, out = self._forward_backward(input_tensor, truth_tensor)
+        finally:
+            hold, self._hold = self._hold, False
+        held, self._held = self._held, None
         self._finish_backward()
         loss_copy = None
         if not self.sync_loss and isinstance(self.optim, FlatAdamW) and loss.is_cuda:
             loss_copy = torch.empty_like(loss)
             self.optim.copy_scalar = (loss.detach(), loss_copy)
-        self.optim.step()
-        if loss_copy is not None and self.optim.copy_scalar is not None:
-            self.optim.copy_scalar = None
-            loss_copy = None
-        self.model.invalidate_packed_weights()
+        if held is not None and self.optim.finish_step(held, self.model.packed_convs()):
+            self._packed_at = self.optim.flat_version()
+            self.model.invalidate_half_weights()
+        else:
+            if held is not None:
+                held.reduce_only()
+            if hold:
+                self.finish_in_reduction = False
+                self.dp_schedule["step_finish"] = "reduction, optimizer launch, repack in the next prologue (the finishing launch did not apply)"
+            self.optim.step()
+            if loss_copy is not None and self.optim.copy_scalar is not None:
+                self.optim.copy_scalar = None
+                loss_copy = None
+            self.model.invalidate_packed_weights()
 
         if self.global_step == 1:
             self.validate_for_train(args, val_dataloader)
@@ -656,6 +708,13 @@
             return loss.item()
         self._loss_in_flight = False
         return loss_copy if loss_copy is not None else loss.detach().clone()
+
+    def _finish_applies(self, input_tensor):
+        return (self.finish_in_reduction and input_tensor.is_cuda and isinstance(self.optim, FlatAdamW)
+                and self.grad_bucket is not None and self.grad_bucket.intact(self.model) and self.optim.flat_version() is not None)
+
+    def _packed_images_stale(self):
+        return self.model.packed_weights_stale() or self._packed_at != self.optim.flat_version()
 
     def _poll_loss(self):
         cell = self._handoffs["poll"]
diff --git a/larvanet_amd/optim.py b/larvanet_amd/optim.py
--- a/larvanet_amd/optim.py
+++ b/larvanet_amd/optim.py
@@ -54,6 +54,27 @@
                           g["eps"], g["weight_decay"], self.mean_scale, copy=copy)
         return None
 
+    def flat_version(self):
+        return None if self._flat_p is None else self._flat_p._version
+
+    @torch.no_grad()
+    def finish_step(self, held, pcs):
+        if len(self.param_groups) != 1 or not self._flat_ok():
+            return False
+        g = self.param_groups[0]
+        if g.get("amsgrad") or g.get("maximize"):
+            return False
+        launch = held.finisher(pcs, self._bucket.flat, self._flat_p, self._m, self._v)
+        if launch is None:
+            return False
+        b1, b2 = g["betas"]
+        if not launch.launch(self._t + 1, float(g["lr"]), b1, b2, g["eps"], g["weight_decay"], self.mean_scale,
+                             copy=self.copy_scalar):
+            return False
+        self._t += 1
+        self.copy_scalar = None
+        return True
+
     def training_state(self):
         if self._flat_p is not None:
             return {"flat": True, "t": self._t, "m": self._m.detach().cpu().clone(), "v": self._v.detach().cpu().clone(),
```

Result: no change. 362.5 HR Mpixels/s (median of 3 runs) (-0.1%).
